# tum-pbs/DMCF

Hardware: AMD Instinct MI355X
Metric: rollout_particle_steps_per_sec (higher is better)
Workload: dtype f32

## Files before the change

dmcf_amd/_lib.py:

```python
import ctypes
import os
import subprocess

_PKG = os.path.dirname(os.path.abspath(__file__))
LIB_PATH = os.path.join(_PKG, "libdmcf_hip.so")
_lib = None


class DmcfError(RuntimeError):
    pass


class CconvArgs(ctypes.Structure):
    _fields_ = [
        ("filters", ctypes.c_void_p),
        ("filter_dims", ctypes.c_int32 * 5),
        ("sym_axis", ctypes.c_int32),
        ("out_positions", ctypes.c_void_p),
        ("n_out", ctypes.c_int64),
        ("inp_positions", ctypes.c_void_p),
        ("n_inp", ctypes.c_int64),
        ("inp_features", ctypes.c_void_p),
        ("inp_importance", ctypes.c_void_p),
        ("neighbors_index", ctypes.c_void_p),
        ("neighbors_row_splits", ctypes.c_void_p),
        ("neighbors_value", ctypes.c_void_p),
        ("extent", ctypes.c_float),
        ("window_fac", ctypes.c_float),
        ("window", ctypes.c_int32),
        ("coordinate_mapping", ctypes.c_int32),
        ("interpolation", ctypes.c_int32),
        ("flags", ctypes.c_int32),
        ("bias", ctypes.c_void_p),
        ("out", ctypes.c_void_p),
        ("n_pairs", ctypes.c_int64),
        ("neighbors_row_count", ctypes.c_void_p),
        ("filter_tile_mask", ctypes.c_uint32),
        ("row_length_hint", ctypes.c_int32),
    ]


class CconvBackwardArgs(ctypes.Structure):
    _fields_ = [
        ("struct_size", ctypes.c_uint32),
        ("flags", ctypes.c_int32),
        ("grad_out", ctypes.c_void_p),
        ("inv_index", ctypes.c_void_p),
        ("inv_pair", ctypes.c_void_p),
        ("inv_row_splits", ctypes.c_void_p),
        ("inv_n_rows", ctypes.c_int64),
        ("inv_n_pairs", ctypes.c_int64),
        ("grad_filters", ctypes.c_void_p),
        ("grad_inp_features", ctypes.c_void_p),
    ]


class NeighborDenseArgs(ctypes.Structure):
    _fields_ = [
        ("struct_size", ctypes.c_uint32),
        ("flags", ctypes.c_int32),
        ("x", ctypes.c_void_p),
        ("n_in", ctypes.c_int64),
        ("cin", ctypes.c_int32),
        ("cout", ctypes.c_int32),
        ("kernel", ctypes.c_void_p),
        ("bias", ctypes.c_void_p),
        ("residual", ctypes.c_void_p),
        ("mask", ctypes.c_void_p),
        ("neighbors_index", ctypes.c_void_p),
        ("neighbors_row_splits", ctypes.c_void_p),
        ("neighbors_row_count", ctypes.c_void_p),
        ("n_out", ctypes.c_int64),
        ("n_pairs", ctypes.c_int64),
        ("host_row_splits", ctypes.c_void_p),
        ("out", ctypes.c_void_p),
        ("record_s", ctypes.c_void_p),
        ("record_count", ctypes.c_void_p),
    ]


class NeighborDenseBackwardArgs(ctypes.Structure):
    _fields_ = [
        ("struct_size", ctypes.c_uint32),
        ("flags", ctypes.c_int32),
        ("x", ctypes.c_void_p),
        ("n_in", ctypes.c_int64),
        ("cin", ctypes.c_int32),
        ("cout", ctypes.c_int32),
        ("kernel", ctypes.c_void_p),
        ("grad_out", ctypes.c_void_p),
        ("n_out", ctypes.c_int64),
        ("s", ctypes.c_void_p),
        ("count", ctypes.c_void_p),
        ("inv_index", ctypes.c_void_p),
        ("inv_row_splits", ctypes.c_void_p),
        ("inv_n_pairs", ctypes.c_int64),
        ("grad_x", ctypes.c_void_p),
        ("grad_kernel", ctypes.c_void_p),
        ("grad_bias", ctypes.c_void_p),
    ]


class LatticeConvArgs(ctypes.Structure):
    _fields_ = [
        ("filters", ctypes.c_void_p),
        ("filter_dims", ctypes.c_int32 * 5),
        ("inp_volume", ctypes.c_void_p),
        ("inp_min", ctypes.c_int32 * 3),
        ("inp_dims", ctypes.c_int32 * 3),
        ("out_table", ctypes.c_void_p),
        ("out_min", ctypes.c_int32 * 3),
        ("out_dims", ctypes.c_int32 * 3),
        ("n_out", ctypes.c_int64),
        ("inp_step", ctypes.c_int32),
        ("out_stride", ctypes.c_int32),
        ("out_phase", ctypes.c_int32 * 3),
        ("base_min", ctypes.c_int32 * 3),
        ("base_dims", ctypes.c_int32 * 3),
        ("rel_shift", ctypes.c_float * 3),
        ("voxel", ctypes.c_float * 3),
        ("offsets", ctypes.c_void_p),
        ("n_offsets", ctypes.c_int64),
        ("reach", ctypes.c_int32 * 3),
        ("extent", ctypes.c_float),
        ("window_fac", ctypes.c_float),
        ("window", ctypes.c_int32),
        ("coordinate_mapping", ctypes.c_int32),
        ("interpolation", ctypes.c_int32),
        ("flags", ctypes.c_int32),
        ("bias", ctypes.c_void_p),
        ("out", ctypes.c_void_p),
    ]


class CconvScatterArgs(ctypes.Structure):
    _fields_ = [
        ("filters", ctypes.c_void_p),
        ("filter_dims", ctypes.c_int32 * 5),
        ("out_positions", ctypes.c_void_p),
        ("n_out", ctypes.c_int64),
        ("inp_positions", ctypes.c_void_p),
        ("n_inp", ctypes.c_int64),
        ("inp_features", ctypes.c_void_p),
        ("t_index", ctypes.c_void_p),
        ("t_row_begin", ctypes.c_void_p),
        ("t_row_count", ctypes.c_void_p),
        ("t_capacity", ctypes.c_int64),
        ("plan", ctypes.c_void_p),
        ("block_cells", ctypes.c_int32),
        ("reach", ctypes.c_int32),
        ("extent", ctypes.c_float),
        ("window_fac", ctypes.c_float),
        ("window", ctypes.c_int32),
        ("flags", ctypes.c_int32),
        ("bias", ctypes.c_void_p),
        ("out", ctypes.c_void_p),
        ("error_flag", ctypes.c_void_p),
    ]


class AdamTensor(ctypes.Structure):
    _fields_ = [
        ("param", ctypes.c_void_p),
        ("grad", ctypes.c_void_p),
        ("m", ctypes.c_void_p),
        ("v", ctypes.c_void_p),
        ("n", ctypes.c_int64),
    ]


class AdamArgs(ctypes.Structure):
    _fields_ = [
        ("struct_size", ctypes.c_uint32),
        ("n_tensors", ctypes.c_int32),
        ("tensors", ctypes.c_void_p),
        ("device_tensors", ctypes.c_void_p),
        ("lr", ctypes.c_float),
        ("beta_1", ctypes.c_float),
        ("beta_2", ctypes.c_float),
        ("epsilon", ctypes.c_float),
        ("beta_1_power", ctypes.c_float),
        ("beta_2_power", ctypes.c_float),
        ("clip_norm", ctypes.c_float),
        ("reserved", ctypes.c_int32),
    ]


class Sph1dParams(ctypes.Structure):
    _fields_ = [
        ("struct_size", ctypes.c_uint32),
        ("bcnt", ctypes.c_int32),
        ("max_iter", ctypes.c_int32),
        ("reserved", ctypes.c_int32),
        ("h", ctypes.c_double),
        ("rest_dens", ctypes.c_double),
        ("stiffness", ctypes.c_double),
        ("visc", ctypes.c_double),
        ("gravity", ctypes.c_double),
        ("dt", ctypes.c_double),
        ("eps", ctypes.c_double),
    ]


SYMBOLS = [
    "dmcf_version", "dmcf_error_string", "dmcf_last_hip_error",
    "dmcf_frs_workspace_bytes", "dmcf_frs_build", "dmcf_frs_count", "dmcf_frs_write", "dmcf_frs_search_padded", "dmcf_frs_window_sum",
    "dmcf_radius_search_count", "dmcf_radius_search_write",
    "dmcf_cconv_workspace_bytes", "dmcf_cconv_forward", "dmcf_cconv_kernel_name",
    "dmcf_cconv_forward_extents", "dmcf_cconv_extents_kernel_name",
    "dmcf_invert_neighbors_list_workspace_bytes", "dmcf_invert_neighbors_list",
    "dmcf_cconv_backward_workspace_bytes", "dmcf_cconv_backward", "dmcf_cconv_backward_kernel_names",
    "dmcf_cconv_backward_extents", "dmcf_cconv_backward_extents_kernel_names",
    "dmcf_cconv_scatter_plan_bytes", "dmcf_cconv_scatter_plan", "dmcf_cconv_scatter_workspace_bytes", "dmcf_cconv_scatter_forward",
    "dmcf_lattice_conv_workspace_bytes", "dmcf_lattice_conv_forward",
    "dmcf_lattice_conv_batch_workspace_bytes", "dmcf_lattice_conv_forward_batch",
    "dmcf_lattice_conv_backward_workspace_bytes", "dmcf_lattice_conv_backward",
    "dmcf_reduce_subarrays_sum", "dmcf_points_aabb_workspace_bytes", "dmcf_points_aabb", "dmcf_dense_forward",
    "dmcf_fps_workspace_bytes", "dmcf_farthest_point_sample", "dmcf_gather_point",
    "dmcf_grid_pos_workspace_bytes", "dmcf_grid_pos_bounds", "dmcf_grid_pos_count", "dmcf_grid_pos_write",
    "dmcf_ghost_workspace_bytes", "dmcf_ghost_count", "dmcf_ghost_write",
    "dmcf_nn_distance_workspace_bytes", "dmcf_nn_distance", "dmcf_approx_match_workspace_bytes", "dmcf_approx_match",
    "dmcf_match_cost_workspace_bytes", "dmcf_match_cost", "dmcf_emd_workspace_bytes", "dmcf_emd",
    "dmcf_neighbor_dense_forward", "dmcf_neighbor_dense_backward_workspace_bytes", "dmcf_neighbor_dense_backward",
    "dmcf_neighbor_dense_kernel_names", "dmcf_adam_step_workspace_bytes", "dmcf_adam_step", "dmcf_adam_step_kernel_names",
    "dmcf_raster_workspace_bytes", "dmcf_raster_count", "dmcf_raster_discs",
    "dmcf_nn_distance_backward_workspace_bytes", "dmcf_nn_distance_backward", "dmcf_match_cost_backward_workspace_bytes",
    "dmcf_match_cost_backward", "dmcf_emd_with_levels", "dmcf_emd_backward_workspace_bytes", "dmcf_emd_backward",
    "dmcf_gather_point_backward_workspace_bytes", "dmcf_gather_point_backward",
    "dmcf_frs_window_sum_backward",
    "dmcf_sph1d_rollout",
]


def build(force=False):
    csrc = os.path.join(_PKG, "csrc")
    args = ["make", "-C", csrc, "-j4"]
    if force:
        args.append("-B")
    subprocess.check_call(args, stdout=subprocess.DEVNULL)
    return LIB_PATH


def lib():
    global _lib
    if _lib is not None:
        return _lib
    if not os.path.exists(LIB_PATH):
        raise DmcfError(
            f"{LIB_PATH} is missing: the HIP extension has not been built "
            "(run `python -c 'import __graft_entry__ as g; g.build()'`). There is no CPU fallback.")
    L = ctypes.CDLL(LIB_PATH)
    c = ctypes
    L.dmcf_version.restype = c.c_int
    L.dmcf_error_string.restype = c.c_char_p
    L.dmcf_error_string.argtypes = [c.c_int]
    L.dmcf_last_hip_error.restype = c.c_int
    L.dmcf_frs_workspace_bytes.restype = c.c_size_t
    L.dmcf_frs_workspace_bytes.argtypes = [c.c_int64, c.c_int64]
    L.dmcf_frs_build.restype = c.c_int
    L.dmcf_frs_build.argtypes = [c.c_void_p, c.c_int64, c.c_float, c.c_void_p, c.c_size_t, c.c_void_p]
    L.dmcf_frs_count.restype = c.c_int
    L.dmcf_frs_count.argtypes = [c.c_void_p, c.c_int64, c.c_int64, c.c_float, c.c_int, c.c_void_p, c.c_size_t,
                                 c.c_void_p, c.c_void_p]
    L.dmcf_frs_write.restype = c.c_int
    L.dmcf_frs_write.argtypes = [c.c_void_p, c.c_int64, c.c_int64, c.c_float, c.c_int, c.c_void_p, c.c_size_t,
                                 c.c_void_p, c.c_void_p, c.c_void_p, c.c_int64, c.c_void_p]
    L.dmcf_frs_search_padded.restype = c.c_int
    L.dmcf_frs_search_padded.argtypes = [c.c_void_p, c.c_int64, c.c_int64, c.c_float, c.c_int, c.c_void_p, c.c_size_t, c.c_int64,
                                         c.c_void_p, c.c_void_p, c.c_void_p, c.c_void_p, c.c_void_p, c.c_void_p]
    L.dmcf_frs_window_sum.restype = c.c_int
    L.dmcf_frs_window_sum.argtypes = [c.c_void_p, c.c_int64, c.c_int64, c.c_float, c.c_int, c.c_int, c.c_void_p, c.c_size_t,
                                      c.c_void_p, c.c_void_p]
    L.dmcf_radius_search_count.restype = c.c_int
    L.dmcf_radius_search_count.argtypes = [c.c_void_p, c.c_int64, c.c_int64, c.c_void_p, c.c_float, c.c_int, c.c_void_p, c.c_size_t,
                                           c.c_void_p, c.c_void_p]
    L.dmcf_radius_search_write.restype = c.c_int
    L.dmcf_radius_search_write.argtypes = [c.c_void_p, c.c_int64, c.c_int64, c.c_void_p, c.c_float, c.c_int, c.c_void_p, c.c_size_t,
                                           c.c_void_p, c.c_void_p, c.c_void_p, c.c_int64, c.c_void_p]
    L.dmcf_cconv_workspace_bytes.restype = c.c_size_t
    L.dmcf_cconv_workspace_bytes.argtypes = [c.POINTER(CconvArgs)]
    L.dmcf_cconv_forward.restype = c.c_int
    L.dmcf_cconv_forward.argtypes = [c.POINTER(CconvArgs), c.c_void_p, c.c_size_t, c.c_void_p]
    L.dmcf_cconv_kernel_name.restype = c.c_int
    L.dmcf_cconv_kernel_name.argtypes = [c.POINTER(CconvArgs), c.c_char_p, c.c_size_t]
    L.dmcf_cconv_forward_extents.restype = c.c_int
    L.dmcf_cconv_forward_extents.argtypes = [c.POINTER(CconvArgs), c.c_void_p, c.c_void_p, c.c_size_t, c.c_void_p]
    L.dmcf_cconv_extents_kernel_name.restype = c.c_int
    L.dmcf_cconv_extents_kernel_name.argtypes = [c.POINTER(CconvArgs), c.c_char_p, c.c_size_t]
    L.dmcf_invert_neighbors_list_workspace_bytes.restype = c.c_size_t
    L.dmcf_invert_neighbors_list_workspace_bytes.argtypes = [c.c_int64]
    L.dmcf_invert_neighbors_list.restype = c.c_int
    L.dmcf_invert_neighbors_list.argtypes = [c.c_int64, c.c_void_p, c.c_void_p, c.c_void_p, c.c_int64, c.c_int64, c.c_void_p,
                                             c.c_void_p, c.c_void_p, c.c_void_p, c.c_void_p, c.c_void_p, c.c_size_t, c.c_void_p]
    L.dmcf_cconv_backward_workspace_bytes.restype = c.c_size_t
    L.dmcf_cconv_backward_workspace_bytes.argtypes = [c.POINTER(CconvArgs), c.POINTER(CconvBackwardArgs)]
    L.dmcf_cconv_backward.restype = c.c_int
    L.dmcf_cconv_backward.argtypes = [c.POINTER(CconvArgs), c.POINTER(CconvBackwardArgs), c.c_void_p, c.c_size_t, c.c_void_p]
    L.dmcf_cconv_backward_kernel_names.restype = c.c_int
    L.dmcf_cconv_backward_kernel_names.argtypes = [c.POINTER(CconvArgs), c.POINTER(CconvBackwardArgs), c.c_char_p, c.c_size_t]
    L.dmcf_cconv_backward_extents.restype = c.c_int
    L.dmcf_cconv_backward_extents.argtypes = [c.POINTER(CconvArgs), c.POINTER(CconvBackwardArgs), c.c_void_p, c.c_void_p, c.c_size_t,
                                              c.c_void_p]
    L.dmcf_cconv_backward_extents_kernel_names.restype = c.c_int
    L.dmcf_cconv_backward_extents_kernel_names.argtypes = [c.POINTER(CconvArgs), c.POINTER(CconvBackwardArgs), c.c_char_p, c.c_size_t]
    L.dmcf_cconv_scatter_plan_bytes.restype = c.c_size_t
    L.dmcf_cconv_scatter_plan_bytes.argtypes = [c.c_int64]
    L.dmcf_cconv_scatter_plan.restype = c.c_int
    L.dmcf_cconv_scatter_plan.argtypes = [c.c_void_p, c.c_int64, c.c_void_p, c.c_int64, c.c_float, c.c_float, c.c_int32, c.c_void_p,
                                          c.c_size_t, c.c_void_p]
    L.dmcf_cconv_scatter_workspace_bytes.restype = c.c_size_t
    L.dmcf_cconv_scatter_workspace_bytes.argtypes = [c.POINTER(CconvScatterArgs)]
    L.dmcf_cconv_scatter_forward.restype = c.c_int
    L.dmcf_cconv_scatter_forward.argtypes = [c.POINTER(CconvScatterArgs), c.c_void_p, c.c_size_t, c.c_void_p]
    L.dmcf_lattice_conv_workspace_bytes.restype = c.c_size_t
    L.dmcf_lattice_conv_workspace_bytes.argtypes = [c.POINTER(LatticeConvArgs)]
    L.dmcf_lattice_conv_forward.restype = c.c_int
    L.dmcf_lattice_conv_forward.argtypes = [c.POINTER(LatticeConvArgs), c.c_void_p, c.c_size_t, c.c_void_p]
    L.dmcf_lattice_conv_batch_workspace_bytes.restype = c.c_size_t
    L.dmcf_lattice_conv_batch_workspace_bytes.argtypes = [c.POINTER(LatticeConvArgs), c.c_int32]
    L.dmcf_lattice_conv_forward_batch.restype = c.c_int
    L.dmcf_lattice_conv_forward_batch.argtypes = [c.POINTER(LatticeConvArgs), c.c_int32, c.c_void_p, c.c_size_t, c.c_void_p]
    L.dmcf_lattice_conv_backward_workspace_bytes.restype = c.c_size_t
    L.dmcf_lattice_conv_backward_workspace_bytes.argtypes = [c.POINTER(LatticeConvArgs), c.c_int32]
    L.dmcf_lattice_conv_backward.restype = c.c_int
    L.dmcf_lattice_conv_backward.argtypes = [c.POINTER(LatticeConvArgs), c.c_int32, c.c_void_p, c.c_void_p, c.c_void_p, c.c_void_p,
                                             c.c_size_t, c.c_void_p]
    L.dmcf_dense_forward.restype = c.c_int
    L.dmcf_dense_forward.argtypes = [c.c_void_p, c.c_int64, c.c_int32, c.c_void_p, c.c_int32, c.c_void_p, c.c_void_p, c.c_void_p,
                                     c.c_void_p]
    L.dmcf_ghost_workspace_bytes.restype = c.c_size_t
    L.dmcf_ghost_workspace_bytes.argtypes = [c.c_int64, c.c_int32, c.c_int32]
    L.dmcf_ghost_count.restype = c.c_int
    L.dmcf_ghost_count.argtypes = [c.c_void_p, c.c_int64, c.c_void_p, c.c_int32, c.c_void_p, c.c_int32, c.c_void_p, c.c_void_p,
                                   c.c_size_t, c.c_void_p]
    L.dmcf_ghost_write.restype = c.c_int
    L.dmcf_ghost_write.argtypes = [c.c_void_p, c.c_int64, c.c_void_p, c.c_int32, c.c_void_p, c.c_int32, c.c_void_p, c.c_void_p,
                                   c.c_void_p, c.c_void_p, c.c_size_t, c.c_void_p]
    L.dmcf_points_aabb_workspace_bytes.restype = c.c_size_t
    L.dmcf_points_aabb_workspace_bytes.argtypes = []
    L.dmcf_points_aabb.restype = c.c_int
    L.dmcf_points_aabb.argtypes = [c.c_void_p, c.c_int64, c.c_void_p, c.c_void_p, c.c_size_t, c.c_void_p]
    L.dmcf_reduce_subarrays_sum.restype = c.c_int
    L.dmcf_reduce_subarrays_sum.argtypes = [c.c_void_p, c.c_void_p, c.c_int64, c.c_void_p, c.c_void_p]
    L.dmcf_fps_workspace_bytes.restype = c.c_size_t
    L.dmcf_fps_workspace_bytes.argtypes = [c.c_int64]
    L.dmcf_farthest_point_sample.restype = c.c_int
    L.dmcf_farthest_point_sample.argtypes = [c.c_void_p, c.c_int64, c.c_int64, c.c_void_p, c.c_size_t, c.c_void_p, c.c_void_p]
    L.dmcf_gather_point.restype = c.c_int
    L.dmcf_gather_point.argtypes = [c.c_void_p, c.c_void_p, c.c_int64, c.c_int, c.c_void_p, c.c_void_p]
    L.dmcf_grid_pos_workspace_bytes.restype = c.c_size_t
    L.dmcf_grid_pos_workspace_bytes.argtypes = [c.c_int64]
    f3 = c.POINTER(c.c_float)
    L.dmcf_grid_pos_bounds.restype = c.c_int
    L.dmcf_grid_pos_bounds.argtypes = [c.c_void_p, c.c_int64, f3, c.c_int, c.c_void_p, c.c_int, c.c_float, c.c_void_p,
                                       c.c_size_t, c.c_void_p]
    L.dmcf_grid_pos_count.restype = c.c_int
    L.dmcf_grid_pos_count.argtypes = [c.c_void_p, c.c_int64, f3, c.c_int, c.c_int, c.c_float, c.c_void_p, c.c_size_t,
                                      c.c_void_p, c.c_int64, c.c_void_p]
    L.dmcf_grid_pos_write.restype = c.c_int
    L.dmcf_grid_pos_write.argtypes = [c.c_void_p, c.c_int64, f3, c.c_int, c.c_int, c.c_float, c.c_void_p, c.c_size_t,
                                      c.c_void_p, c.c_int64, c.c_void_p, c.c_int64, c.c_void_p]
    for q in ("dmcf_nn_distance_workspace_bytes", "dmcf_approx_match_workspace_bytes", "dmcf_match_cost_workspace_bytes",
              "dmcf_emd_workspace_bytes"):
        getattr(L, q).restype = c.c_size_t
        getattr(L, q).argtypes = [c.c_int64, c.c_int64, c.c_int64]
    L.dmcf_nn_distance.restype = c.c_int
    L.dmcf_nn_distance.argtypes = [c.c_void_p, c.c_void_p, c.c_int64, c.c_int64, c.c_int64, c.c_void_p, c.c_void_p, c.c_void_p,
                                   c.c_void_p, c.c_void_p, c.c_size_t, c.c_void_p]
    i32p = c.POINTER(c.c_int32)
    for f in ("dmcf_approx_match", "dmcf_emd"):
        getattr(L, f).restype = c.c_int
        getattr(L, f).argtypes = [c.c_void_p, c.c_void_p, c.c_int64, c.c_int64, c.c_int64, i32p, i32p, c.c_void_p, c.c_void_p,
                                  c.c_size_t, c.c_void_p]
    L.dmcf_match_cost.restype = c.c_int
    L.dmcf_match_cost.argtypes = [c.c_void_p, c.c_void_p, c.c_int64, c.c_int64, c.c_int64, c.c_void_p, c.c_void_p, c.c_void_p,
                                  c.c_size_t, c.c_void_p]
    L.dmcf_neighbor_dense_forward.restype = c.c_int
    L.dmcf_neighbor_dense_forward.argtypes = [c.POINTER(NeighborDenseArgs), c.c_void_p]
    L.dmcf_neighbor_dense_backward_workspace_bytes.restype = c.c_size_t
    L.dmcf_neighbor_dense_backward_workspace_bytes.argtypes = [c.POINTER(NeighborDenseBackwardArgs)]
    L.dmcf_neighbor_dense_backward.restype = c.c_int
    L.dmcf_neighbor_dense_backward.argtypes = [c.POINTER(NeighborDenseBackwardArgs), c.c_void_p, c.c_size_t, c.c_void_p]
    L.dmcf_neighbor_dense_kernel_names.restype = c.c_int
    L.dmcf_neighbor_dense_kernel_names.argtypes = [c.POINTER(NeighborDenseArgs), c.POINTER(NeighborDenseBackwardArgs), c.c_char_p,
                                                   c.c_size_t]
    L.dmcf_adam_step_workspace_bytes.restype = c.c_size_t
    L.dmcf_adam_step_workspace_bytes.argtypes = [c.POINTER(AdamArgs)]
    L.dmcf_adam_step.restype = c.c_int
    L.dmcf_adam_step.argtypes = [c.POINTER(AdamArgs), c.c_void_p, c.c_size_t, c.c_void_p]
    L.dmcf_adam_step_kernel_names.restype = c.c_int
    L.dmcf_adam_step_kernel_names.argtypes = [c.POINTER(AdamArgs), c.c_char_p, c.c_size_t]
    L.dmcf_raster_workspace_bytes.restype = c.c_size_t
    L.dmcf_raster_workspace_bytes.argtypes = [c.c_int64, c.c_int64, c.c_int64, c.c_int32, c.c_int32]
    L.dmcf_raster_count.restype = c.c_int
    L.dmcf_raster_count.argtypes = [c.c_void_p, c.c_int64, c.c_int64, c.c_int64, c.c_float, c.c_int32, c.c_int32, c.c_void_p, c.c_size_t,
                                    c.c_void_p, c.c_void_p]
    L.dmcf_raster_discs.restype = c.c_int
    L.dmcf_raster_discs.argtypes = [c.c_void_p, c.c_int64, c.c_int64, c.c_int64, c.c_float, c.c_uint32, c.c_int32, c.c_int32, c.c_void_p,
                                    c.c_void_p, c.c_size_t, c.c_void_p, c.c_int64, c.c_void_p]
    for q in ("dmcf_nn_distance_backward_workspace_bytes", "dmcf_match_cost_backward_workspace_bytes",
              "dmcf_emd_backward_workspace_bytes"):
        getattr(L, q).restype = c.c_size_t
        getattr(L, q).argtypes = [c.c_int64, c.c_int64, c.c_int64]
    L.dmcf_nn_distance_backward.restype = c.c_int
    L.dmcf_nn_distance_backward.argtypes = [c.c_void_p, c.c_void_p, c.c_int64, c.c_int64, c.c_int64, c.c_void_p, c.c_void_p,
                                            c.c_void_p, c.c_void_p, c.c_void_p, c.c_void_p, c.c_void_p, c.c_size_t, c.c_void_p]
    L.dmcf_match_cost_backward.restype = c.c_int
    L.dmcf_match_cost_backward.argtypes = [c.c_void_p, c.c_void_p, c.c_int64, c.c_int64, c.c_int64, c.c_void_p, c.c_void_p,
                                           c.c_void_p, c.c_void_p, c.c_void_p, c.c_size_t, c.c_void_p]
    L.dmcf_emd_with_levels.restype = c.c_int
    L.dmcf_emd_with_levels.argtypes = [c.c_void_p, c.c_void_p, c.c_int64, c.c_int64, c.c_int64, i32p, i32p, c.c_void_p, c.c_void_p,
                                       c.c_void_p, c.c_size_t, c.c_void_p]
    L.dmcf_emd_backward.restype = c.c_int
    L.dmcf_emd_backward.argtypes = [c.c_void_p, c.c_void_p, c.c_int64, c.c_int64, c.c_int64, i32p, i32p, c.c_void_p, c.c_void_p,
                                    c.c_void_p, c.c_void_p, c.c_void_p, c.c_size_t, c.c_void_p]
    L.dmcf_gather_point_backward_workspace_bytes.restype = c.c_size_t
    L.dmcf_gather_point_backward_workspace_bytes.argtypes = [c.c_int64, c.c_int64]
    L.dmcf_gather_point_backward.restype = c.c_int
    L.dmcf_gather_point_backward.argtypes = [c.c_void_p, c.c_void_p, c.c_int64, c.c_int, c.c_int64, c.c_void_p, c.c_void_p,
                                             c.c_size_t, c.c_void_p]
    L.dmcf_frs_window_sum_backward.restype = c.c_int
    L.dmcf_frs_window_sum_backward.argtypes = [c.c_void_p, c.c_int64, c.c_int64, c.c_float, c.c_int, c.c_int, c.c_void_p, c.c_void_p,
                                               c.c_void_p, c.c_size_t, c.c_void_p, c.c_void_p]
    L.dmcf_sph1d_rollout.restype = c.c_int
    L.dmcf_sph1d_rollout.argtypes = [c.c_void_p, c.c_void_p, c.c_int64, c.c_int32, c.POINTER(Sph1dParams), c.c_int32, c.c_void_p,
                                     c.c_void_p, c.c_void_p, c.c_void_p]
    _lib = L
    return L


def check(rc, what):
    if rc != 0:
        L = lib()
        raise DmcfError(f"{what}: {L.dmcf_error_string(rc).decode()} (code {rc}, hip error {L.dmcf_last_hip_error()})")
```

dmcf_amd/csrc/cconv_lat.hip:

```cpp
#include "cconv_common.h"

namespace dmcf {

struct LatParams {
    const float* Wp;
    const int32_t* stencil;
    int S, KS, NT, cin, cout;
    const float* vol;
    int imin[3], idim[3];
    const int32_t* otab;
    int omin[3], odim[3];
    int inp_step, out_stride, phase[3];
    int amin[3], adim[3];
    int tiles_x;
    int64_t ntiles;
    const float* bias;
    float* out;
    int flags;
};

typedef int lat_i32x2 __attribute__((ext_vector_type(2)));
constexpr int kLatMaxParts = 8;
constexpr int kLatRowsPerGroup = 128;
constexpr int kLatCellsPerBlock = 1024;
struct LatBatch {
    LatParams part[kLatMaxParts];
    int64_t cfirst[kLatMaxParts + 1];
    int n;
    uint32_t* blk;
    int64_t* start;
    int64_t* count;
    lat_i32x2* rows;
    int64_t rows_capacity;
};

__device__ __forceinline__ int lat_cell(const LatParams& p, int64_t c, int& rowb) {
    const int64_t tile = c >> 4;
    const int m = (int)(c & 15);
    rowb = 0;
    if (tile >= p.ntiles) return -1;
    const int xb = (int)(tile % p.tiles_x);
    const int ax = p.amin[0] + xb * 16 + m, ay = p.amin[1] + (int)(tile / p.tiles_x % p.adim[1]),
              az = p.amin[2] + (int)(tile / ((int64_t)p.tiles_x * p.adim[1]));
    const int ox = ax * p.out_stride + p.phase[0] - p.omin[0], oy = ay * p.out_stride + p.phase[1] - p.omin[1],
              oz = az * p.out_stride + p.phase[2] - p.omin[2];
    if (!(xb * 16 + m < p.adim[0] && (unsigned)ox < (unsigned)p.odim[0] && (unsigned)oy < (unsigned)p.odim[1] &&
          (unsigned)oz < (unsigned)p.odim[2]))
        return -1;
    const int ix = ax * p.inp_step - p.imin[0], iy = ay * p.inp_step - p.imin[1], iz = az * p.inp_step - p.imin[2];
    rowb = ((iz * p.idim[1] + iy) * p.idim[0] + ix) * p.cin * 4;
    return p.otab[((int64_t)oz * p.odim[1] + oy) * p.odim[0] + ox];
}

__device__ __forceinline__ int lat_part_of_block(const LatBatch& b, int64_t block) {
    int i = 0;
    while (i + 1 < b.n && block >= b.cfirst[i + 1]) ++i;
    return i;
}

__global__ __launch_bounds__(256) void lat_rows_count(const LatBatch b) {
    __shared__ uint32_t wsum[4];
    const int i = lat_part_of_block(b, blockIdx.x);
    const int64_t c0 = ((int64_t)blockIdx.x - b.cfirst[i]) * kLatCellsPerBlock;
    uint32_t mine = 0;
    for (int r = 0; r < kLatCellsPerBlock / 256; ++r) {
        int rowb;
        mine += (uint32_t)__popcll(__ballot(lat_cell(b.part[i], c0 + r * 256 + threadIdx.x, rowb) >= 0));
    }
    if ((threadIdx.x & 63) == 0) wsum[threadIdx.x >> 6] = mine;
    __syncthreads();
    if (threadIdx.x == 0) {
        b.blk[blockIdx.x] = wsum[0] + wsum[1] + wsum[2] + wsum[3];
        if (blockIdx.x == 0) b.blk[b.cfirst[b.n]] = 0;
    }
}

__global__ void lat_rows_starts(const LatBatch b) {
    if (threadIdx.x != 0) return;
    int64_t s = 0;
    for (int i = 0; i < b.n; ++i) {
        const int64_t n = (int64_t)b.blk[b.cfirst[i + 1]] - (int64_t)b.blk[b.cfirst[i]];
        b.start[i] = s;
        b.count[i] = n;
        s += (n + kLatRowsPerGroup - 1) / kLatRowsPerGroup * kLatRowsPerGroup;
    }
    b.start[b.n] = s;
}

__global__ __launch_bounds__(256) void lat_rows_write(const LatBatch b) {
    __shared__ uint32_t wsum[4];
    const int i = lat_part_of_block(b, blockIdx.x);
    const int64_t c0 = ((int64_t)blockIdx.x - b.cfirst[i]) * kLatCellsPerBlock;
    const int lane = threadIdx.x & 63, wave = threadIdx.x >> 6;
    int64_t at = b.start[i] + ((int64_t)b.blk[blockIdx.x] - (int64_t)b.blk[b.cfirst[i]]);
    for (int r = 0; r < kLatCellsPerBlock / 256; ++r) {
        int rowb;
        const int oi = lat_cell(b.part[i], c0 + r * 256 + threadIdx.x, rowb);
        const uint64_t mk = __ballot(oi >= 0);
        if (lane == 0) wsum[wave] = (uint32_t)__popcll(mk);
        __syncthreads();
        if (oi >= 0) {
            int64_t pos = at + __popcll(mk & ((1ull << lane) - 1ull));
            for (int v = 0; v < wave; ++v) pos += wsum[v];
            if (pos < b.rows_capacity) b.rows[pos] = (lat_i32x2){rowb, oi};
        }
        at += wsum[0] + wsum[1] + wsum[2] + wsum[3];
        __syncthreads();
    }
}

struct LatTaps {
    float a;
    int bx, by, bz;
    float wx[2], wy[2], wz[2];
};
__device__ __forceinline__ LatTaps lat_offset_taps(const int32_t* __restrict__ stencil, int s, const CconvParams& p, float vx, float vy,
                                                   float vz, float sx, float sy, float sz) {
    LatTaps g;
    float x = (float)stencil[4 * s] * vx - sx, y = (float)stencil[4 * s + 1] * vy - sy, z = (float)stencil[4 * s + 2] * vz - sz;
    const float d2 = (x * x + y * y) + z * z;
    g.a = window_value(p.window, d2, p.inv_r2, p.window_fac);
    filter_coords<true>(x, y, z, p);
    axis_weights(x, p.sx, p.interp, g.bx, g.wx[0], g.wx[1]);
    axis_weights(y, p.sy, p.interp, g.by, g.wy[0], g.wy[1]);
    axis_weights(z, p.sz, p.interp, g.bz, g.wz[0], g.wz[1]);
    return g;
}

__global__ __launch_bounds__(256) void lat_build_filters(const float* __restrict__ W, float* __restrict__ Wp,
                                                         const int32_t* __restrict__ stencil, int S, int KS, int NT, CconvParams p,
                                                         float vx, float vy, float vz, float sx, float sy, float sz) {
    const int64_t total = (int64_t)((S + 3) / 4) * 4 * KS * NT * 64;
    for (int64_t e = (int64_t)blockIdx.x * blockDim.x + threadIdx.x; e < total; e += (int64_t)gridDim.x * blockDim.x) {
        int64_t t = e;
        const int n = (int)(t & 15); t >>= 4;
        const int q = (int)(t & 3); t >>= 2;
        const int nt = (int)(t % NT); t /= NT;
        const int c = (int)(t % (4 * KS)); t /= 4 * KS;
        const int s = (int)t * 4 + q, o = nt * 16 + n;
        float v = 0.0f;
        if (s < S && c < p.cin && o < p.cout) {
            const LatTaps g = lat_offset_taps(stencil, s, p, vx, vy, vz, sx, sy, sz);
            for (int iz = 0; iz < 2; ++iz)
                for (int iy = 0; iy < 2; ++iy)
                    for (int ix = 0; ix < 2; ++ix) {
                        const float w = g.wz[iz] * g.wy[iy] * g.wx[ix];
                        if (w == 0.0f) continue;
                        const int cz = min(g.bz + iz, p.sz - 1), cy = min(g.by + iy, p.sy - 1), cx = min(g.bx + ix, p.sx - 1);
                        v += w * W[((((int64_t)cz * p.sy + cy) * p.sx + cx) * p.cin + c) * p.cout + o];
                    }
            v *= g.a;
        }
        Wp[e] = v;
    }
}

constexpr int kLatTW = 2;
constexpr int kLatCH = 32;
constexpr int kLatG = kLatCH / 4;
static_assert(kLatRowsPerGroup == 4 * kLatTW * 16, "rows of a workgroup");

template <int NTT, int KST>
__device__ __forceinline__ void lat_conv_body(const LatParams& p, const lat_i32x2* __restrict__ rows, const int64_t first, const int64_t end) {
    __shared__ __attribute__((aligned(16))) float Ws[2][kLatCH * KST * NTT * 64];
    const int lane = threadIdx.x & 63, wave = threadIdx.x >> 6;
    const int m = lane & 15, q = lane >> 4;
    constexpr int C = 4 * KST;
    int oidx[kLatTW];
    int rowb[kLatTW];
    f32x4 acc[kLatTW][NTT];
    bool any = false;
#pragma unroll
    for (int t = 0; t < kLatTW; ++t) {
        const int64_t e = first + ((wave * kLatTW + t) << 4) + m;
        oidx[t] = -1;
        rowb[t] = (((p.amin[2] * p.inp_step - p.imin[2]) * p.idim[1] + (p.amin[1] * p.inp_step - p.imin[1])) * p.idim[0] +
                   (p.amin[0] * p.inp_step - p.imin[0])) * p.cin * 4;
        if (e < end) {
            const lat_i32x2 rw = rows[e];
            rowb[t] = rw.x;
            oidx[t] = rw.y;
        }
        if (__ballot(oidx[t] >= 0) == 0) oidx[t] = -2;
        any |= oidx[t] != -2;
#pragma unroll
        for (int n = 0; n < NTT; ++n) acc[t][n] = (f32x4){0.0f, 0.0f, 0.0f, 0.0f};
    }
    if (!__syncthreads_or(any ? 1 : 0)) return;
    typedef int i32x4 __attribute__((ext_vector_type(4)));
    const int NG = (p.S + 3) / 4;
    constexpr int kQuads = kLatCH * KST * NTT * 64 / 4 / 256;
    f32x4 wr[kQuads];
    i32x4 dv;
    auto fetch = [&](int s0) {
        const int g0 = s0 / 4, ng = min(kLatG, NG - g0);
#pragma unroll
        for (int i = 0; i < kQuads; ++i) {
            const int e = (threadIdx.x + 256 * i) * 4;
            const int l = e & 63, n = (e >> 6) % NTT, gc = (e >> 6) / NTT;
            wr[i] = (gc < ng * C && n < p.NT) ? *(const f32x4*)(p.Wp + (((int64_t)g0 * C + gc) * p.NT + n) * 64 + l)
                                              : (f32x4){0.0f, 0.0f, 0.0f, 0.0f};
        }
        dv = *(const i32x4*)(p.stencil + 4 * min(s0 + (lane & (kLatCH - 1)), p.S - 1));
    };
    auto stash = [&](int buf) {
#pragma unroll
        for (int i = 0; i < kQuads; ++i) *(f32x4*)(Ws[buf] + (threadIdx.x + 256 * i) * 4) = wr[i];
    };
    fetch(0);
    stash(0);
    __syncthreads();
    for (int s0 = 0, k = 0; s0 < p.S; s0 += kLatCH, ++k) {
        const int ng = min(kLatG, NG - s0 / 4);
        const float* Wc = Ws[k & 1];
        const int dof = ((dv.z * p.idim[1] + dv.y) * p.idim[0] + dv.x) * p.cin * 4;
        int dofg[kLatG];
#pragma unroll
        for (int g = 0; g < kLatG; ++g) dofg[g] = __shfl(dof, 4 * g + q, 64);
        const bool more = s0 + kLatCH < p.S;
        if (more) fetch(s0 + kLatCH);
        if (any) {
            f32x4 f[3][kLatTW][KST];
            auto gather = [&](int g, f32x4 (&fv)[kLatTW][KST]) {
#pragma unroll
                for (int t = 0; t < kLatTW; ++t) {
                    const f32x4* src = (const f32x4*)((const char*)p.vol + (size_t)(uint32_t)(rowb[t] + dofg[g]));
#pragma unroll
                    for (int ks = 0; ks < KST; ++ks) fv[t][ks] = src[ks];
                }
            };
            auto products = [&](int g, const f32x4 (&fv)[kLatTW][KST]) {
#pragma unroll
                for (int c = 0; c < C; ++c)
#pragma unroll
                    for (int n = 0; n < NTT; ++n) {
                        const float w = Wc[((g * C + c) * NTT + n) * 64 + lane];
#pragma unroll
                        for (int t = 0; t < kLatTW; ++t)
                            acc[t][n] = __builtin_amdgcn_mfma_f32_16x16x4f32(fv[t][c >> 2][c & 3], w, acc[t][n], 0, 0, 0);
                    }
            };
            gather(0, f[0]);
            gather(1, f[1]);
#pragma unroll
            for (int g = 0; g < kLatG; ++g) {
                if (g >= ng) break;
                if (g + 2 < kLatG) gather(g + 2, f[(g + 2) % 3]);
                products(g, f[g % 3]);
            }
        }
        if (more) stash((k + 1) & 1);
        __syncthreads();
    }
#pragma unroll
    for (int t = 0; t < kLatTW; ++t) {
        if (oidx[t] == -2) continue;
#pragma unroll
        for (int r = 0; r < 4; ++r) {
            const int oi = __shfl(oidx[t], 4 * q + r, 64);
            if (oi < 0) continue;
#pragma unroll
            for (int n = 0; n < NTT; ++n) {
                const int o = 16 * n + m;
                if (o >= p.cout) continue;
                float v = acc[t][n][r];
                if (p.bias) v += p.bias[o];
                float* dst = p.out + (int64_t)oi * p.cout + o;
                if (p.flags & DMCF_FLAG_ACCUMULATE) v += *dst;
                *dst = v;
            }
        }
    }
}

template <int NTT, int KST>
__global__ __launch_bounds__(256) void lat_conv_kernel(const LatBatch b) {
    const int64_t first = (int64_t)blockIdx.x * kLatRowsPerGroup;
    if (first >= b.start[b.n]) return;
    int i = 0;
    while (i + 1 < b.n && first >= b.start[i + 1]) ++i;
    lat_conv_body<NTT, KST>(b.part[i], b.rows, first, b.start[i] + b.count[i]);
}

static size_t lat_packed_floats(const dmcf_lattice_conv_args* a) {
    const int KS = (a->filter_dims[3] + 3) / 4, NT = (a->filter_dims[4] + 15) / 16;
    return (size_t)((a->n_offsets + 3) / 4) * 4 * KS * NT * 64;
}

static int lat_validate(const dmcf_lattice_conv_args* a) {
    if (!a) return DMCF_EINVAL;
    for (int k = 0; k < 5; ++k)
        if (a->filter_dims[k] <= 0) return DMCF_EINVAL;
    if (a->n_out < 0 || a->n_offsets < 0 || a->inp_step <= 0 || a->out_stride <= 0 || !(a->extent > 0.0f)) return DMCF_EINVAL;
    if (a->n_out > 0 && (!a->filters || !a->out_table || !a->out || !a->inp_volume || (a->n_offsets > 0 && !a->offsets)))
        return DMCF_EINVAL;
    for (int k = 0; k < 3; ++k)
        if (a->inp_dims[k] <= 0 || a->out_dims[k] <= 0 || a->base_dims[k] <= 0 || !(a->voxel[k] >= 0.0f)) return DMCF_EINVAL;
    if (a->flags & (DMCF_FLAG_SYMMETRIC | DMCF_FLAG_NORMALIZE)) return DMCF_EUNSUPPORTED;
    if (a->window == DMCF_WINDOW_EXPLICIT) return DMCF_EUNSUPPORTED;
    const int cin = a->filter_dims[3], cout = a->filter_dims[4];
    if ((cin != 4 && cin != 8) || cout > 32) return DMCF_EUNSUPPORTED;
    return DMCF_OK;
}

}

namespace dmcf {

static CconvParams lat_cconv_params(const dmcf_lattice_conv_args* a) {
    CconvParams cp = {};
    cp.sz = a->filter_dims[0]; cp.sy = a->filter_dims[1]; cp.sx = a->filter_dims[2];
    cp.K = cp.sx * cp.sy * cp.sz;
    cp.cin = a->filter_dims[3]; cp.cout = a->filter_dims[4];
    cp.inv_extent = 1.0f / a->extent;
    const float radius = 0.5f * a->extent;
    cp.inv_r2 = 1.0f / (radius * radius);
    cp.window_fac = a->window_fac;
    cp.window = a->window;
    cp.mapping = a->coordinate_mapping;
    cp.interp = a->interpolation;
    cp.flags = a->flags;
    return cp;
}

static int lat_prepare(const dmcf_lattice_conv_args* a, float* packed, hipStream_t stream, LatParams& p, int64_t& groups) {
    const int cin = a->filter_dims[3], cout = a->filter_dims[4];
    const int KS = (cin + 3) / 4, NT = (cout + 15) / 16;
    for (int k = 0; k < 3; ++k) {
        const int64_t ext = k == 0 ? (int64_t)((a->base_dims[0] + 15) / 16) * 16 : a->base_dims[k];
        const int64_t lo = (int64_t)a->base_min[k] * a->inp_step - a->reach[k];
        const int64_t hi = ((int64_t)a->base_min[k] + ext - 1) * a->inp_step + a->reach[k];
        if (a->reach[k] < 0 || lo < a->inp_min[k] || hi > (int64_t)a->inp_min[k] + a->inp_dims[k] - 1) return DMCF_EINVAL;
    }
    if ((int64_t)a->inp_dims[0] * a->inp_dims[1] * a->inp_dims[2] * cin > 0x1fffffff) return DMCF_EUNSUPPORTED;
    const CconvParams cp = lat_cconv_params(a);
    if (a->n_offsets > 0) {
        const int64_t total = (int64_t)lat_packed_floats(a);
        const unsigned g = (unsigned)((total + 255) / 256);
        hipLaunchKernelGGL(lat_build_filters, dim3(g < 4096u ? g : 4096u), dim3(256), 0, stream, a->filters, packed, a->offsets,
                           (int)a->n_offsets, KS, NT, cp, a->voxel[0], a->voxel[1], a->voxel[2], a->rel_shift[0], a->rel_shift[1],
                           a->rel_shift[2]);
    }
    p.Wp = packed;
    p.stencil = a->offsets;
    p.S = (int)a->n_offsets; p.KS = KS; p.NT = NT; p.cin = cin; p.cout = cout;
    p.vol = a->inp_volume;
    p.otab = a->out_table;
    for (int k = 0; k < 3; ++k) {
        p.imin[k] = a->inp_min[k]; p.idim[k] = a->inp_dims[k];
        p.omin[k] = a->out_min[k]; p.odim[k] = a->out_dims[k];
        p.phase[k] = a->out_phase[k];
        p.amin[k] = a->base_min[k];
        p.adim[k] = a->base_dims[k];
    }
    p.inp_step = a->inp_step;
    p.out_stride = a->out_stride;
    p.tiles_x = (a->base_dims[0] + 15) / 16;
    p.ntiles = (int64_t)p.tiles_x * a->base_dims[1] * a->base_dims[2];
    p.bias = a->bias; p.out = a->out; p.flags = a->flags;
    groups = (p.ntiles * 16 + kLatCellsPerBlock - 1) / kLatCellsPerBlock;
    return DMCF_OK;
}

struct LatLayout {
    size_t off_blk, off_scan, off_tmp, tmp_bytes, off_start, off_rows, total;
    int64_t nblk, rows_capacity;
};

static LatLayout lat_layout(const dmcf_lattice_conv_args* parts, int n_parts) {
    LatLayout L;
    size_t off = 256;
    L.nblk = 0;
    for (int i = 0; i < n_parts; ++i) {
        off += align_up(lat_packed_floats(parts + i) * sizeof(float), 256);
        const int64_t cells = (int64_t)((parts[i].base_dims[0] + 15) / 16) * 16 * parts[i].base_dims[1] * parts[i].base_dims[2];
        L.nblk += (cells + kLatCellsPerBlock - 1) / kLatCellsPerBlock;
    }
    L.off_blk = off;    off += align_up((size_t)(L.nblk + 1) * 4, 256);
    L.off_scan = off;   off += align_up((size_t)(L.nblk + 1) * 4, 256);
    L.tmp_bytes = scan_tmp_bytes(L.nblk + 1);
    L.off_tmp = off;    off += align_up(L.tmp_bytes, 256);
    L.off_start = off;  off += 256;
    L.rows_capacity = (parts[0].n_out + kLatRowsPerGroup - 1) / kLatRowsPerGroup * kLatRowsPerGroup + (int64_t)kLatRowsPerGroup * n_parts;
    L.off_rows = off;   off += align_up((size_t)L.rows_capacity * sizeof(lat_i32x2), 256);
    L.total = off;
    return L;
}

static int lat_check(const dmcf_lattice_conv_args* parts, int n_parts) {
    for (int i = 0; i < n_parts; ++i) {
        const int rc = lat_validate(parts + i);
        if (rc != DMCF_OK) return rc;
        if (parts[i].filter_dims[3] != parts[0].filter_dims[3] || parts[i].filter_dims[4] != parts[0].filter_dims[4] ||
            parts[i].n_out != parts[0].n_out || parts[i].out != parts[0].out)
            return DMCF_EINVAL;
    }
    return DMCF_OK;
}

static int lat_rows(const dmcf_lattice_conv_args* parts, int n_parts, void* workspace, size_t workspace_bytes, size_t need,
                    hipStream_t stream, LatBatch& b, const LatLayout& L) {
    if (!workspace || ((uintptr_t)workspace & 255)) return DMCF_EINVAL;
    if (workspace_bytes < need) return DMCF_EWORKSPACE;
    if (L.nblk > 0x7ffffffe) return DMCF_EUNSUPPORTED;
    b.n = n_parts;
    char* ws = (char*)workspace;
    char* wp = ws;
    int64_t first = 0;
    for (int i = 0; i < n_parts; ++i) {
        int64_t blocks;
        const int rc = lat_prepare(parts + i, (float*)wp, stream, b.part[i], blocks);
        if (rc != DMCF_OK) return rc;
        wp += align_up(lat_packed_floats(parts + i) * sizeof(float), 256);
        b.cfirst[i] = first;
        first += blocks;
    }
    for (int i = n_parts; i <= kLatMaxParts; ++i) b.cfirst[i] = first;
    if (first != L.nblk) return DMCF_EINVAL;
    uint32_t* blk_in = (uint32_t*)(ws + L.off_blk);
    b.blk = blk_in;
    b.start = (int64_t*)(ws + L.off_start);
    b.count = b.start + kLatMaxParts + 1;
    b.rows = (lat_i32x2*)(ws + L.off_rows);
    b.rows_capacity = L.rows_capacity;
    hipLaunchKernelGGL(lat_rows_count, dim3((unsigned)L.nblk), dim3(256), 0, stream, b);
    const int rc = scan_exclusive_u32(blk_in, (uint32_t*)(ws + L.off_scan), L.nblk + 1, ws + L.off_tmp, L.tmp_bytes, stream);
    if (rc != DMCF_OK) return rc;
    b.blk = (uint32_t*)(ws + L.off_scan);
    hipLaunchKernelGGL(lat_rows_starts, dim3(1), dim3(64), 0, stream, b);
    hipLaunchKernelGGL(lat_rows_write, dim3((unsigned)L.nblk), dim3(256), 0, stream, b);
    return DMCF_OK;
}

static int lat_launch(const dmcf_lattice_conv_args* parts, int n_parts, void* workspace, size_t workspace_bytes, hipStream_t stream) {
    int rc = lat_check(parts, n_parts);
    if (rc != DMCF_OK) return rc;
    if (parts[0].n_out == 0) return DMCF_OK;
    const LatLayout L = lat_layout(parts, n_parts);
    LatBatch b;
    rc = lat_rows(parts, n_parts, workspace, workspace_bytes, L.total, stream, b, L);
    if (rc != DMCF_OK) return rc;
    const dim3 grid((unsigned)(L.rows_capacity / kLatRowsPerGroup)), block(256);
    const int KS = b.part[0].KS, NT = b.part[0].NT;
    if (KS == 1 && NT == 1) hipLaunchKernelGGL((lat_conv_kernel<1, 1>), grid, block, 0, stream, b);
    else if (KS == 1) hipLaunchKernelGGL((lat_conv_kernel<2, 1>), grid, block, 0, stream, b);
    else if (NT == 1) hipLaunchKernelGGL((lat_conv_kernel<1, 2>), grid, block, 0, stream, b);
    else hipLaunchKernelGGL((lat_conv_kernel<2, 2>), grid, block, 0, stream, b);
    return check_launch();
}

#include "cconv_lat_bwd.inc"

}

using namespace dmcf;

extern "C" {

size_t dmcf_lattice_conv_workspace_bytes(const dmcf_lattice_conv_args* a) {
    if (lat_validate(a) != DMCF_OK) return 256;
    return lat_layout(a, 1).total;
}

size_t dmcf_lattice_conv_batch_workspace_bytes(const dmcf_lattice_conv_args* parts, int32_t n_parts) {
    if (!parts || n_parts < 1 || n_parts > kLatMaxParts) return 256;
    for (int i = 0; i < n_parts; ++i)
        if (lat_validate(parts + i) != DMCF_OK) return 256;
    return lat_layout(parts, n_parts).total;
}

int dmcf_lattice_conv_forward(const dmcf_lattice_conv_args* a, void* workspace, size_t workspace_bytes, dmcf_stream_t stream_) {
    if (!a) return DMCF_EINVAL;
    return lat_launch(a, 1, workspace, workspace_bytes, (hipStream_t)stream_);
}

int dmcf_lattice_conv_forward_batch(const dmcf_lattice_conv_args* parts, int32_t n_parts, void* workspace, size_t workspace_bytes,
                                    dmcf_stream_t stream_) {
    if (!parts || n_parts < 1 || n_parts > kLatMaxParts) return DMCF_EINVAL;
    return lat_launch(parts, n_parts, workspace, workspace_bytes, (hipStream_t)stream_);
}

size_t dmcf_lattice_conv_backward_workspace_bytes(const dmcf_lattice_conv_args* parts, int32_t n_parts) {
    dmcf_lattice_conv_args own[kLatMaxParts];
    if (lat_bwd_parts(parts, n_parts, own) != DMCF_OK) return 256;
    return lat_bwd_layout(own, n_parts).total;
}

int dmcf_lattice_conv_backward(const dmcf_lattice_conv_args* parts, int32_t n_parts, const float* grad_out, float* grad_volume,
                               float* grad_filters, void* workspace, size_t workspace_bytes, dmcf_stream_t stream_) {
    return lat_backward(parts, n_parts, grad_out, grad_volume, grad_filters, workspace, workspace_bytes, (hipStream_t)stream_);
}

}
```

dmcf_amd/csrc/misc.hip:

```cpp
#include "common.h"

namespace dmcf {

thread_local int g_last_hip_error = 0;

constexpr int kScanThreads = 256;
constexpr int kScanItems = 8;
constexpr int kScanTile = kScanThreads * kScanItems;

template <typename T>
__device__ __forceinline__ T wave_inclusive_scan(T v) {
#pragma unroll
    for (int d = 1; d < kWave; d <<= 1) {
        T o = __shfl_up(v, d, kWave);
        if (lane_id() >= d) v += o;
    }
    return v;
}

template <typename T>
__device__ __forceinline__ T block_exclusive_scan(T v, T* total, T* smem ) {
    const int wave = threadIdx.x >> 6;
    const T inc = wave_inclusive_scan(v);
    if (lane_id() == kWave - 1) smem[wave] = inc;
// ... 88 lines not shown
int scan_exclusive_u32(const uint32_t* in, uint32_t* out, int64_t n, void* tmp, size_t tmp_bytes,
                       hipStream_t stream) {
    return scan_impl<uint32_t, uint32_t, false>(in, out, n, tmp, tmp_bytes, stream);
}

int scan_counts_to_row_splits(const int32_t* counts, int64_t* row_splits, int64_t n, void* tmp,
                              size_t tmp_bytes, hipStream_t stream) {
    return scan_impl<int32_t, int64_t, true>(counts, row_splits, n, tmp, tmp_bytes, stream);
}

typedef float dense_f32x4 __attribute__((ext_vector_type(4)));
template <int NT>
__global__ __launch_bounds__(256) void dense_rows(const float* __restrict__ x, int64_t n, int k, const float* __restrict__ W, int m,
                                                  const float* __restrict__ bias, const float* __restrict__ residual,
                                                  float* __restrict__ out, int64_t ntiles) {
    const int lane = lane_id(), r = lane & 15, q = lane >> 4;
    const int kj = (k + 15) >> 4;
    float wf[4][4][NT];
#pragma unroll
    for (int j = 0; j < 4; ++j)
#pragma unroll
        for (int i = 0; i < 4; ++i)
#pragma unroll
            for (int t = 0; t < NT; ++t) {
                const int kk = 16 * j + 4 * q + i, col = 16 * t + r;
                wf[j][i][t] = (kk < k && col < m) ? W[(size_t)kk * m + col] : 0.0f;
            }
    float bs[NT];
#pragma unroll
    for (int t = 0; t < NT; ++t) bs[t] = (bias && 16 * t + r < m) ? bias[16 * t + r] : 0.0f;
    const int64_t wave = (int64_t)blockIdx.x * 4 + (threadIdx.x >> 6), nwaves = (int64_t)gridDim.x * 4;
    for (int64_t tile = wave; tile < ntiles; tile += nwaves) {
        const int64_t row = tile * 16 + r;
        dense_f32x4 a[4];
#pragma unroll
        for (int j = 0; j < 4; ++j) {
            a[j] = (dense_f32x4){0.0f, 0.0f, 0.0f, 0.0f};
            if (j < kj && row < n && 16 * j + 4 * q < k) a[j] = *(const dense_f32x4*)(x + row * k + 16 * j + 4 * q);
        }
        dense_f32x4 acc[NT];
#pragma unroll
        for (int t = 0; t < NT; ++t) acc[t] = (dense_f32x4){0.0f, 0.0f, 0.0f, 0.0f};
#pragma unroll
        for (int j = 0; j < 4; ++j) {
            if (j < kj) {
#pragma unroll
                for (int i = 0; i < 4; ++i)
#pragma unroll
                    for (int t = 0; t < NT; ++t) acc[t] = __builtin_amdgcn_mfma_f32_16x16x4f32(a[j][i], wf[j][i][t], acc[t], 0, 0, 0);
            }
        }
#pragma unroll
        for (int rr = 0; rr < 4; ++rr) {
            const int64_t orow = tile * 16 + 4 * q + rr;
            if (orow >= n) continue;
#pragma unroll
            for (int t = 0; t < NT; ++t) {
                const int col = 16 * t + r;
                if (col >= m) continue;
                float v = acc[t][rr] + bs[t];
                if (residual) v += residual[orow * m + col];
                out[orow * m + col] = v;
            }
        }
    }
}

constexpr int kAabbBlocks = 1024;

__global__ __launch_bounds__(256) void aabb_partial(const float* __restrict__ pts, int64_t n, float* __restrict__ part) {
    float mn[3] = {INFINITY, INFINITY, INFINITY}, mx[3] = {-INFINITY, -INFINITY, -INFINITY};
    bool bad[3] = {false, false, false};
    for (int64_t i = (int64_t)blockIdx.x * 256 + threadIdx.x; i < n; i += (int64_t)gridDim.x * 256) {
#pragma unroll
        for (int a = 0; a < 3; ++a) {
            const float v = pts[3 * i + a];
            mn[a] = fminf(mn[a], v);
            mx[a] = fmaxf(mx[a], v);
            bad[a] |= v != v;
        }
    }
    __shared__ float red[3][3][4];
#pragma unroll
    for (int a = 0; a < 3; ++a) {
        float b = bad[a] ? 1.0f : 0.0f;
#pragma unroll
        for (int d = 32; d >= 1; d >>= 1) {
            mn[a] = fminf(mn[a], __shfl_xor(mn[a], d, kWave));
            mx[a] = fmaxf(mx[a], __shfl_xor(mx[a], d, kWave));
            b = fmaxf(b, __shfl_xor(b, d, kWave));
        }
        if (lane_id() == 0) {
            red[0][a][threadIdx.x >> 6] = mn[a];
            red[1][a][threadIdx.x >> 6] = mx[a];
            red[2][a][threadIdx.x >> 6] = b;
        }
    }
    __syncthreads();
    if (threadIdx.x < 3) {
        const int a = threadIdx.x;
        float* o = part + (size_t)blockIdx.x * 8;
        const bool b = fmaxf(fmaxf(red[2][a][0], red[2][a][1]), fmaxf(red[2][a][2], red[2][a][3])) > 0.0f;
        o[a] = b ? NAN : fminf(fminf(red[0][a][0], red[0][a][1]), fminf(red[0][a][2], red[0][a][3]));
        o[3 + a] = b ? NAN : fmaxf(fmaxf(red[1][a][0], red[1][a][1]), fmaxf(red[1][a][2], red[1][a][3]));
    }
}

__global__ void aabb_finish(const float* __restrict__ part, int nblocks, float* __restrict__ out) {
    const int lane = lane_id();
#pragma unroll
    for (int a = 0; a < 3; ++a) {
        float mn = INFINITY, mx = -INFINITY, b = 0.0f;
        for (int k = lane; k < nblocks; k += kWave) {
            const float lo = part[(size_t)k * 8 + a], hi = part[(size_t)k * 8 + 3 + a];
            b = fmaxf(b, lo != lo ? 1.0f : 0.0f);
            mn = fminf(mn, lo);
            mx = fmaxf(mx, hi);
        }
#pragma unroll
        for (int d = 32; d >= 1; d >>= 1) {
            mn = fminf(mn, __shfl_xor(mn, d, kWave));
            mx = fmaxf(mx, __shfl_xor(mx, d, kWave));
            b = fmaxf(b, __shfl_xor(b, d, kWave));
        }
        if (lane == 0) {
            out[a] = b > 0.0f ? NAN : mn;
            out[3 + a] = b > 0.0f ? NAN : mx;
        }
    }
}

__global__ __launch_bounds__(256) void reduce_subarrays_sum_kernel(const float* __restrict__ values,
                                                                   const int64_t* __restrict__ row_splits,
                                                                   int64_t n_rows, float* __restrict__ out) {
    const int64_t row = ((int64_t)blockIdx.x * blockDim.x + threadIdx.x) >> 4;
    const int sub = threadIdx.x & 15;
    if (row >= n_rows) return;
    const int64_t b = row_splits[row], e = row_splits[row + 1];
    float s = 0.0f;
    if (values) {
        for (int64_t k = b + sub; k < e; k += 16) s += values[k];
    } else {
        for (int64_t k = b + sub; k < e; k += 16) s += 1.0f;
    }
#pragma unroll
    for (int d = 8; d >= 1; d >>= 1) s += __shfl_xor(s, d, 16);
    if (sub == 0) out[row] = s;
}

}

extern "C" {

int dmcf_version(void) { return 21700; }

const char* dmcf_error_string(int code) {
    switch (code) {
        case DMCF_OK: return "ok";
        case DMCF_EINVAL: return "invalid argument";
        case DMCF_EWORKSPACE: return "workspace too small";
        case DMCF_ELAUNCH: return "HIP error while enqueuing (see dmcf_last_hip_error)";
        case DMCF_EUNSUPPORTED: return "option not implemented on the HIP path";
        default: return "unknown error code";
    }
}

int dmcf_last_hip_error(void) { return dmcf::g_last_hip_error; }

int dmcf_dense_forward(const float* x, int64_t n, int32_t k, const float* W, int32_t m, const float* bias,
                       const float* residual, float* out, dmcf_stream_t stream) {
    if (n < 0 || k <= 0 || m <= 0 || (n > 0 && (!x || !W || !out))) return DMCF_EINVAL;
    if ((k & 3) || k > 64 || m > 64) return DMCF_EUNSUPPORTED;
    if ((uintptr_t)x & 15) return DMCF_EUNSUPPORTED;
    if (n == 0) return DMCF_OK;
    const int64_t ntiles = (n + 15) / 16;
    const int64_t want = (ntiles + 3) / 4;
    const unsigned grid = (unsigned)(want < 2048 ? want : 2048);
    const int nt = (m + 15) / 16;
#define DMCF_DENSE(NTT)                                                                                                   \
    hipLaunchKernelGGL(dmcf::dense_rows<NTT>, dim3(grid), dim3(256), 0, (hipStream_t)stream, x, n, (int)k, W, (int)m, bias,  \
                       residual, out, ntiles)
    if (nt <= 1) DMCF_DENSE(1);
    else if (nt == 2) DMCF_DENSE(2);
    else DMCF_DENSE(4);
#undef DMCF_DENSE
    return dmcf::check_launch();
}

size_t dmcf_points_aabb_workspace_bytes(void) { return (size_t)dmcf::kAabbBlocks * 8 * sizeof(float); }

int dmcf_points_aabb(const float* points, int64_t n, float* out, void* workspace, size_t workspace_bytes,
                     dmcf_stream_t stream) {
    if (n < 0 || !out || (n > 0 && !points)) return DMCF_EINVAL;
    if (!workspace || workspace_bytes < dmcf_points_aabb_workspace_bytes()) return DMCF_EWORKSPACE;
    const int64_t want = (n + 1023) / 1024;
    const int nb = (int)(want < 1 ? 1 : (want > dmcf::kAabbBlocks ? dmcf::kAabbBlocks : want));
    hipLaunchKernelGGL(dmcf::aabb_partial, dim3(nb), dim3(256), 0, (hipStream_t)stream, points, n, (float*)workspace);
    hipLaunchKernelGGL(dmcf::aabb_finish, dim3(1), dim3(64), 0, (hipStream_t)stream, (const float*)workspace, nb, out);
    return dmcf::check_launch();
}

int dmcf_reduce_subarrays_sum(const float* values, const int64_t* row_splits, int64_t n_rows, float* out,
                              dmcf_stream_t stream) {
    if (n_rows < 0 || (n_rows > 0 && (!row_splits || !out))) return DMCF_EINVAL;
    if (n_rows == 0) return DMCF_OK;
    const int64_t threads = n_rows * 16;
    const unsigned grid = (unsigned)((threads + 255) / 256);
    hipLaunchKernelGGL(dmcf::reduce_subarrays_sum_kernel, dim3(grid), dim3(256), 0, (hipStream_t)stream, values,
                       row_splits, n_rows, out);
    return dmcf::check_launch();
}

}
```

dmcf_amd/lattice.py:

```python
import collections
import os
import threading

import numpy as np
import torch

_TLS = threading.local()
_KEEP = 16

MAX_X_OVER_EXTENT = float(os.environ.get("DMCF_LATTICE_MAX_RATIO", "32"))
MAX_VOLUME_FLOATS = 1 << 28
MAX_CELLS_PER_POINT = 32
CORE_MIN_FILL = float(os.environ.get("DMCF_LATTICE_CORE_FILL", str(1.0 / 32)))
CORE_SLAB_FRACTION = 0.125
_FAR = 3.0e4


def _registry():
    r = getattr(_TLS, "registry", None)
    if r is None:
        r = _TLS.registry = collections.OrderedDict()
    return r


def clear():
    _registry().clear()


def _cores():
    r = getattr(_TLS, "cores", None)
    if r is None:
        r = _TLS.cores = {}
    return r


def _pick_core(minp, dims, hists):
    lo, hi = [], []
    for k in range(3):
        h = hists[k]
        m = max(h) if h else 0
        if m <= 0:
            lo.append(minp[k]); hi.append(minp[k] + dims[k])
            continue
        thr = CORE_SLAB_FRACTION * m
        peak = h.index(m)
        a = b = peak
        gap = 0
        i = peak - 1
        while i >= 0 and gap <= 2:
            if h[i] >= thr:
                a, gap = i, 0
            else:
                gap += 1
            i -= 1
        gap = 0
        i = peak + 1
        while i < len(h) and gap <= 2:
            if h[i] >= thr:
                b, gap = i, 0
            else:
                gap += 1
            i += 1
        lo.append(minp[k] + a); hi.append(minp[k] + b + 1)
    return lo, hi


class LatticeInfo:
    def __init__(self, gpos, center, voxel, family, minp, dims, keep=None, center_host=None):
        self.gpos = gpos
        self.max_abs = None
        if center_host is not None:
            self.max_abs = max(abs(float(center_host[k])) + max(abs(int(minp[k])), abs(int(minp[k]) + int(dims[k]))) * float(voxel[k])
                               for k in range(3))
        self.keep = keep
        self.version = gpos._version
        self.center = center
        self.voxel = tuple(float(np.float32(v)) for v in voxel)
        self.family = family
        self.minp = [int(v) for v in minp]
        self.dims = [int(v) for v in dims]
        self._cells = None
        self._lin = None
        self._vlin = {}
        self._table = None
        self._core = None
        self._tables = {}

    def cells(self):
        if self._cells is None:
            v = torch.tensor(self.voxel, dtype=torch.float32, device=self.gpos.device)
            self._cells = torch.round((self.gpos - self.center) / v).to(torch.int32).contiguous()
        return self._cells

    def lin(self, minp=None, dims=None):
        own = minp is None
        if own and self._lin is not None:
            return self._lin
        minp, dims = (self.minp, self.dims) if own else (minp, dims)
        dx, dy, dz = dims
        c = self.cells().long()
        lin = ((c[:, 2] - minp[2]) * dy + (c[:, 1] - minp[1])) * dx + (c[:, 0] - minp[0])
        if os.environ.get("DMCF_LATTICE_CHECK") == "1":
            lo = torch.tensor(list(minp), device=c.device)
            hi = lo + torch.tensor(list(dims), device=c.device)
            if not bool(((c >= lo) & (c < hi)).all()):
                raise RuntimeError("lattice points outside the registered box of cells")
        if own:
            self._lin = lin
        return lin

    def core(self):
        if self._core is not None:
            return self._core
        n = self.gpos.shape[0]
        dx, dy, dz = self.dims
        whole = (list(self.minp), list(self.dims), None, None, None)
        if n / float(dx * dy * dz) >= CORE_MIN_FILL or os.environ.get("DMCF_LATTICE_CORE", "1") == "0":
            self._core = whole
            return whole
        from .utils.convolutions import _CACHE
        dev = self.gpos.device
        c = self.cells()
        minp, dims = list(self.minp), list(self.dims)
        lo_box = torch.tensor(minp, dtype=torch.int32, device=dev)
        rel = torch.minimum((c - lo_box).long().clamp_(min=0), torch.tensor(dims, device=dev) - 1)
        hist = torch.cat([torch.bincount(rel[:, k], minlength=dims[k])[: dims[k]] for k in range(3)])
        key = (_CACHE.key, self.voxel)

        def split(h):
            return [h[: dx], h[dx: dx + dy], h[dx + dy:]]

        def next_entry(h):
            hs = split(h)
            lo, hi = _pick_core(minp, dims, hs)
            bound = sum(n - sum(hs[k][lo[k] - minp[k]: hi[k] - minp[k]]) for k in range(3))
            return dict(box=(lo, hi), cap=int(2 * bound + 65536))

        est = _cores().get(key) if (_CACHE.depth > 0 and _CACHE.use_hints) else None
        if est is None:
            est = next_entry(hist.tolist())
            exact = True
        else:
            exact = False
        lo = [max(est["box"][0][k], minp[k]) for k in range(3)]
        hi = [min(est["box"][1][k], minp[k] + dims[k]) for k in range(3)]
        if any(hi[k] <= lo[k] for k in range(3)):
            lo, hi = minp, [minp[k] + dims[k] for k in range(3)]
        lo_t = torch.tensor(lo, dtype=torch.int32, device=dev)
        hi_t = torch.tensor(hi, dtype=torch.int32, device=dev)
        outside = ~((c >= lo_t) & (c < hi_t)).all(dim=1)
        count = outside.sum().reshape(1)
        if exact:
            m = int(count.item())
            _cores()[key] = est
            valid = None
        else:
            m = min(est["cap"], n)
            cap = m

            def report(vals):
                _cores()[key] = next_entry(vals[1:])
                return vals[0] > cap
            _CACHE.report(torch.cat([count, hist]), report)
        if m == 0:
            idx = pos = valid = None
        else:
            idx = torch.nonzero_static(outside, size=m, fill_value=-1).flatten()
            if not exact:
                valid = (idx >= 0).to(torch.float32).unsqueeze(1)
                idx = idx.clamp(min=0)
            pos = self.gpos.index_select(0, idx).contiguous()
            if valid is not None:
                far = max(_FAR, 4.0 * (self.max_abs or 0.0) + 1.0e3)
                pos = torch.where(valid > 0, pos, torch.full_like(pos, far))
        self._core = (lo, [hi[k] - lo[k] for k in range(3)], idx, pos, valid)
        return self._core

    def table_in(self, minp, dims):
        key = (tuple(minp), tuple(dims))
        t = self._tables.get(key)
        if t is None:
            dx, dy, dz = dims
            c = self.cells().long()
            lo = torch.tensor(list(minp), device=c.device)
            hi = lo + torch.tensor(list(dims), device=c.device)
            ok = ((c >= lo) & (c < hi)).all(dim=1)
            lin = ((c[:, 2] - minp[2]) * dy + (c[:, 1] - minp[1])) * dx + (c[:, 0] - minp[0])
            lin = torch.where(ok, lin, torch.full_like(lin, dz * dy * dx))
            t = torch.full((dz * dy * dx + 1,), -1, dtype=torch.int32, device=c.device)
            t[lin] = torch.where(ok, torch.arange(c.shape[0], dtype=torch.int32, device=c.device), torch.full((1,), -1, dtype=torch.int32, device=c.device))
            t = self._tables[key] = t[:-1].view(dz, dy, dx)
        return t

    def volume_in(self, features, minp, dims):
        key = ("in", tuple(minp), tuple(dims))
        lin = self._vlin.get(key)
        dx, dy, dz = dims
        if lin is None:
            c = self.cells().long()
            lo = torch.tensor(list(minp), device=c.device)
            hi = lo + torch.tensor(list(dims), device=c.device)
            ok = ((c >= lo) & (c < hi)).all(dim=1)
            lin = ((c[:, 2] - minp[2]) * dy + (c[:, 1] - minp[1])) * dx + (c[:, 0] - minp[0])
            lin = self._vlin[key] = torch.where(ok, lin, torch.full_like(lin, dz * dy * dx))
        v = features.new_zeros((dz * dy * dx + 1, features.shape[1]))
        v[lin] = features
        return v[:-1].view(dz, dy, dx, features.shape[1])

    def table(self):
        if self._table is None:
            dx, dy, dz = self.dims
            t = torch.full((dz * dy * dx,), -1, dtype=torch.int32, device=self.gpos.device)
            t[self.lin()] = torch.arange(self.gpos.shape[0], dtype=torch.int32, device=self.gpos.device)
            self._table = t.view(dz, dy, dx)
        return self._table

    def volume(self, features, minp=None, dims=None):
        key = None if minp is None else (tuple(minp), tuple(dims))
        lin = self._vlin.get(key)
        if lin is None:
            lin = self._vlin[key] = self.lin(minp, dims)
        dx, dy, dz = self.dims if minp is None else dims
        v = features.new_zeros((dz * dy * dx, features.shape[1]))
        v[lin] = features
        return v.view(dz, dy, dx, features.shape[1])


def register(gpos, center, voxel, family, minp, dims, keep=None, center_host=None):
    if gpos.shape[0] == 0 or any(not (float(v) > 1e-5) for v in voxel):
        return
    reg = _registry()
    reg[(gpos.data_ptr(), gpos.shape[0])] = LatticeInfo(gpos, center, voxel, family, minp, dims, keep, center_host)
    while len(reg) > _KEEP:
        reg.popitem(last=False)


def register_points(pos, center, voxel, family, box=None, keep=None, center_host=None):
    if pos.shape[0] == 0 or any(not (float(v) > 1e-5) for v in voxel) or not pos.is_cuda:
        return
    if box is None:
        v = torch.tensor([float(np.float32(x)) for x in voxel], dtype=torch.float32, device=pos.device)
        cells = torch.round((pos - center) / v).to(torch.int32)
        lo, hi = cells.amin(dim=0), cells.amax(dim=0)
        b = torch.cat([lo, hi - lo + 1]).tolist()
        box = (b[0:3], b[3:6])
    info = LatticeInfo(pos, center, voxel, family, box[0], box[1], keep if keep is not None else center, center_host)
    reg = _registry()
    reg[(pos.data_ptr(), pos.shape[0])] = info
    while len(reg) > _KEEP:
        reg.popitem(last=False)


def lookup(t):
    info = _registry().get((t.data_ptr(), t.shape[0]))
    if info is None or info.gpos._version != info.version or t.dim() != 2 or t.dtype != torch.float32 or not t.is_contiguous():
        return None
    return info


def enabled():
    from . import ops
    return os.environ.get("DMCF_LATTICE_CONV", "1") != "0" and ops.search_set() == "distance"


class LatticePair:

    def __init__(self, inp, out, ratio):
        self.inp, self.out, self.ratio = inp, out, ratio

    def plan(self, ops, extent, dev):
        key = (float(extent), str(dev))
        hit = getattr(self, "_plan", None)
        if hit is not None and hit[0] == key:
            return hit[1]
        a, b = self.inp, self.out
        radius = 0.5 * float(extent)
        omin, odim = b.core()[:2]
        cropped = self.cropped = (omin, odim) != (list(b.minp), list(b.dims)) or a.core()[2] is not None
        if self.ratio >= 1:
            step = int(self.ratio)
            if cropped:
                vmin, vdim = ops.lattice_volume_box(omin, odim, step, ops.lattice_reach(a.voxel, radius, dev))
            else:
                vmin, vdim = ops.lattice_volume_box(b.minp, b.dims, step, ops.lattice_reach(a.voxel, radius, dev), a.minp, a.dims)
            res = (vmin, vdim, None)
        else:
            lo = [omin[k] for k in range(3)]
            hi = [omin[k] + odim[k] - 1 for k in range(3)]
            if cropped:
                launches, vlo, vhi = [], [1 << 30] * 3, [-(1 << 30)] * 3
            else:
                launches, vlo, vhi = [], list(a.minp), [a.minp[k] + a.dims[k] - 1 for k in range(3)]
            for pz in (0, 1):
                for py in (0, 1):
                    for px in (0, 1):
                        ph = (px, py, pz)
                        bmin = [-((ph[k] - lo[k]) // 2) for k in range(3)]
                        bmax = [(hi[k] - ph[k]) // 2 for k in range(3)]
                        bdim = [bmax[k] - bmin[k] + 1 for k in range(3)]
                        if min(bdim) <= 0:
                            continue
                        shift = [ph[k] * b.voxel[k] for k in range(3)]
                        m, d = ops.lattice_volume_box(bmin, bdim, 1, ops.lattice_reach(a.voxel, radius, dev, shift))
                        vlo = [min(vlo[k], m[k]) for k in range(3)]
                        vhi = [max(vhi[k], m[k] + d[k] - 1) for k in range(3)]
                        launches.append((ph, bmin, bdim, shift))
            vdim = [vhi[k] - vlo[k] + 1 for k in range(3)]
            parts = [dict(out_phase=ph, rel_shift=shift, base_min=bmin, base_dims=bdim) for ph, bmin, bdim, shift in launches]
            res = (vlo, vdim, parts)
        self._plan = (key, res)
        return res

    def volume_cells(self, ops, extent, dev):
        vdim = self.plan(ops, extent, dev)[1]
        return int(vdim[0]) * int(vdim[1]) * int(vdim[2])

    def conv(self, ops, kernel, inp_features, n_out, extent, **kw):
        a, b = self.inp, self.out
        vmin, vdim, parts = self.plan(ops, extent, inp_features.device)
        if self.cropped:
            omin, odim = b.core()[:2]
            vol, table, tmin = a.volume_in(inp_features, vmin, vdim), b.table_in(omin, odim), omin
            fill = min(1.0, a.gpos.shape[0] / float(max(vdim[0] * vdim[1] * vdim[2], 1)))
        else:
            vol, table, tmin = a.volume(inp_features, vmin, vdim), b.table(), b.minp
            fill = a.gpos.shape[0] / float(a.dims[0] * a.dims[1] * a.dims[2])
        if parts is None:
            return ops.lattice_conv(kernel, vol, vmin, table, tmin, n_out, a.voxel, extent, inp_step=int(self.ratio),
                                    fill=fill, **kw)
        return ops.lattice_conv(kernel, vol, vmin, table, tmin, n_out, a.voxel, extent, inp_step=1, out_stride=2,
                                parts=parts, fill=fill, **kw)

    def strays(self):
        _, _, idx, pos, valid = self.out.core()
        return None if idx is None else (idx, pos, valid)


def pair(inp_positions, out_positions, extent=None):
    if not enabled():
        return None
    a, b = lookup(inp_positions), lookup(out_positions)
    if a is None or b is None or a.family != b.family:
        return None
    if extent is not None:
        if a.max_abs is None or b.max_abs is None or max(a.max_abs, b.max_abs) > MAX_X_OVER_EXTENT * float(extent):
            return None
    if all(a.voxel[k] == 2.0 * b.voxel[k] for k in range(3)):
        return LatticePair(a, b, 0.5)
    step = round(b.voxel[0] / a.voxel[0])
    if step < 1 or any(b.voxel[k] != step * a.voxel[k] for k in range(3)):
        return None
    return LatticePair(a, b, int(step))
```

dmcf_amd/ops.py:

```python
import collections
import os
import ctypes

import threading

import numpy as np
import torch

from . import _lib

class NeighborCapacityExceeded(RuntimeError):
    """A search enqueued with estimated buffer sizes produced more pairs than the buffers hold."""


class NeighborSearchResult:

    def __init__(self, index_buf, row_splits, dist_buf, total=None, redo=None):
        self._index_buf, self._dist_buf = index_buf, dist_buf
        self.neighbors_row_splits = row_splits
        self._total = total
        self._redo = redo

    def raw(self):
        return self._index_buf, self.neighbors_row_splits, self._dist_buf

    def release(self):
        if self._index_buf is not None:
            self._capacity = self._index_buf.shape[0]
        self._index_buf = self._dist_buf = None
        self._redo = None

    @property
    def total_ref(self):
        return self.neighbors_row_splits[-1]

    @property
    def capacity(self):
        return self._index_buf.shape[0] if self._index_buf is not None else self._capacity

    def resolve(self):
        if self._total is None:
            total = int(self.neighbors_row_splits[-1].item())
            if total > self._index_buf.shape[0]:
                self._index_buf, self._dist_buf = self._redo(pair_capacity(total))
            self._total = total
        return self._total

    def overflowed(self, total):
        return self._total is None and total > self.capacity

    @property
    def neighbors_index(self):
        return self._index_buf[:self.resolve()]

    @property
    def neighbors_distance(self):
        n = self.resolve()
        return self._dist_buf[:n] if self._dist_buf.shape[0] >= n else self._dist_buf

    def __iter__(self):
        return iter((self.neighbors_index, self.neighbors_row_splits, self.neighbors_distance))

    def __getitem__(self, i):
        return tuple(self)[i]

    def __len__(self):
        return 3

class PaddedNeighborList(NeighborSearchResult):

    def __init__(self, index_buf, row_begin, dist_buf, counts, max_count, stride, redo_exact):
        super().__init__(index_buf, row_begin, dist_buf, total=None, redo=None)
        self.row_count = counts
        self.max_count = max_count
        self.stride = int(stride)
        self._redo_exact = redo_exact
        self._compact = None

    @property
    def total_ref(self):
        t = getattr(self, "_total_ref", None)
        if t is None:
            small = self.row_count.shape[0] * self.stride < 2 ** 31
            t = self._total_ref = self.row_count.sum(dtype=torch.int32) if small else self.row_count.sum()
        return t

    def release(self):
        super().release()
        self._redo_exact = None
        self._compact = None

    def overflowed(self, max_count):
        return max_count > self.stride

    def resolve(self):
        if self._compact is None:
            if int(self.max_count.item()) > self.stride:
                self._compact = self._redo_exact()
            else:
                m = self.row_count.shape[0]
                cnt = self.row_count.long()
                rs = torch.zeros(m + 1, dtype=torch.int64, device=cnt.device)
                torch.cumsum(cnt, 0, out=rs[1:])
                total = int(rs[-1].item())
                row = torch.repeat_interleave(torch.arange(m, device=cnt.device), cnt, output_size=total)
                src = row * self.stride + (torch.arange(total, device=cnt.device) - rs[:-1][row])
                dist = self._dist_buf[src] if self._dist_buf.shape[0] else self._dist_buf
                self._compact = NeighborSearchResult(self._index_buf[src], rs, dist, total=total)
        return self._compact

    @property
    def neighbors_index(self):
        return self.resolve().neighbors_index

    @property
    def neighbors_distance(self):
        return self.resolve().neighbors_distance

    @property
    def csr_row_splits(self):
        return self.resolve().neighbors_row_splits

    def __iter__(self):
        c = self.resolve()
        return iter((c.neighbors_index, c.neighbors_row_splits, c.neighbors_distance))


MAPPINGS = {"ball_to_cube_radial": 0, "ball_to_cube_volume_preserving": 1, "identity": 2}
INTERPOLATIONS = {"linear": 0, "linear_border": 1, "nearest_neighbor": 2}
WINDOWS = {None: 0, "explicit": 1, "poly6": 2, "cubic": 3, "linear": 4, "peak": 5, "cubic_grad": 6}

FLAG_ALIGN_CORNERS, FLAG_NORMALIZE, FLAG_SYMMETRIC, FLAG_ACCUMULATE, FLAG_SKIP_SELF, FLAG_FILTER_PACKED = 1, 2, 4, 8, 16, 32


class LaunchTimer:

    def __init__(self):
        self.records = []

    def begin(self):
        ev = torch.cuda.Event(enable_timing=True)
        ev.record(torch.cuda.current_stream())
        return ev

    def end(self, kind, meta, start):
        ev = torch.cuda.Event(enable_timing=True)
        ev.record(torch.cuda.current_stream())
        self.records.append((kind, meta, start, ev))

    def results(self):
        out = []
        for k, m, s, e in self.records:
            m = {a: (int(b.item()) if isinstance(b, torch.Tensor) else b) for a, b in m.items()}
            out.append((k, m, s.elapsed_time(e)))
        return out


timer = None


_raw_stream = getattr(torch._C, "_cuda_getCurrentRawStream", None)


def _stream():
    if _raw_stream is not None:
        return ctypes.c_void_p(_raw_stream(torch.cuda.current_device()))
    return ctypes.c_void_p(torch.cuda.current_stream().cuda_stream)


def _dev_f32(t, name, cols=None):
    if not isinstance(t, torch.Tensor):
        raise TypeError(f"{name} must be a torch tensor")
    if not t.is_cuda:
        raise _lib.DmcfError(f"{name} is on {t.device}: the DMCF hot path runs on the GPU only (no CPU fallback)")
    if t.dtype != torch.float32:
        raise TypeError(f"{name} must be float32, got {t.dtype}")
    if cols is not None and (t.dim() != 2 or t.shape[1] != cols):
        raise ValueError(f"{name} must have shape [n,{cols}], got {tuple(t.shape)}")
    t = t.contiguous()
    if t.data_ptr() % 16:
        t = t.clone()
    return t


def _ptr(t):
    return None if t is None else ctypes.c_void_p(t.data_ptr())


class SpatialHashTable:

    def __init__(self, points, radius, workspace, n_queries_capacity):
        self.points = points
        self.radius = float(radius)
        self.workspace = workspace
        self.n_queries_capacity = n_queries_capacity


def build_spatial_hash_table(points, radius, n_queries=None, **_ignored):
    L = _lib.lib()
    points = _dev_f32(points, "points", 3)
    n = points.shape[0]
    m = n if n_queries is None else int(n_queries)
    nbytes = L.dmcf_frs_workspace_bytes(n, m)
    ws = torch.empty(nbytes, dtype=torch.uint8, device=points.device)
    t0 = timer.begin() if timer is not None else None
    _lib.check(L.dmcf_frs_build(_ptr(points), n, float(radius), _ptr(ws), nbytes, _stream()), "dmcf_frs_build")
    if timer is not None:
        timer.end("frs_build", dict(n_points=n), t0)
    return SpatialHashTable(points, radius, ws, m)


def reserve_device_memory(gib, device=None):
    dev = torch.device("cuda", torch.cuda.current_device()) if device is None else torch.device(device)
    before = torch.cuda.memory_stats(dev).get("num_device_alloc", 0)
    try:
        block = torch.empty(int(gib * (1 << 30)), dtype=torch.uint8, device=dev)
    except torch.cuda.OutOfMemoryError:
        return -1.0
    del block
    return float(gib) if torch.cuda.memory_stats(dev).get("num_device_alloc", 0) > before else 0.0


def pair_capacity(total):
    x = int(total) + int(total) // 8 + 65536
    return _size_class(x)


def _size_class(x):
    x = max(int(x), 1)
    if x >= 1 << 27:
        g = 1 << 28
    else:
        g = max(1 << 16, 1 << max(x.bit_length() - 4, 0))
    return (x + g - 1) // g * g


FRS_IGNORE_QUERY_POINT, FRS_OPEN3D_CORNER_VOXELS, FRS_OPEN3D_VOXEL_WALK = 1, 2, 4

SEARCH_SETS = {"distance": 0, "open3d": FRS_OPEN3D_VOXEL_WALK, "open3d_corners": FRS_OPEN3D_CORNER_VOXELS}


_CONSTS = {}


def const_tensor(values, dtype, device):
    key = (tuple(float(v) for v in values), dtype, str(device))
    t = _CONSTS.get(key)
    if t is None:
        if len(_CONSTS) > 256:
            _CONSTS.clear()
        t = _CONSTS[key] = torch.tensor(list(values), dtype=dtype, device=device)
    return t


def search_set():
    if "DMCF_FRS_BRUTE_FORCE_SET" in os.environ:
        raise ValueError("DMCF_FRS_BRUTE_FORCE_SET is gone: use DMCF_FRS_SET=distance (what it selected) | open3d | open3d_corners")
    name = os.environ.get("DMCF_FRS_SET", "distance")
    if name not in SEARCH_SETS:
        raise ValueError(f"DMCF_FRS_SET={name!r}: expected one of {sorted(SEARCH_SETS)}")
    return name


def frs_flags(ignore_query_point):
    return (FRS_IGNORE_QUERY_POINT if ignore_query_point else 0) | SEARCH_SETS[search_set()]


def fixed_radius_search(points, queries, radius, ignore_query_point=False, return_distances=True,
                        hash_table=None, capacity_hint=None, row_stride=None, max_count=None):
    L = _lib.lib()
    points = _dev_f32(points, "points", 3)
    queries = _dev_f32(queries, "queries", 3)
    radius = float(radius)
    if not radius > 0:
        raise ValueError("radius must be positive")
    n, m = points.shape[0], queries.shape[0]
    if hash_table is None or hash_table.n_queries_capacity < m or hash_table.points.data_ptr() != points.data_ptr() \
            or hash_table.radius != radius:
        hash_table = build_spatial_hash_table(points, radius, n_queries=m)
    ws = hash_table.workspace
    nbytes = L.dmcf_frs_workspace_bytes(n, hash_table.n_queries_capacity)
    flags = frs_flags(ignore_query_point)
    dev = points.device
    row_splits = torch.empty(m + 1, dtype=torch.int64, device=dev)
    if row_stride is not None:
# ... 149 lines not shown
        twin = getattr(self, "_index_only", None)
        if twin is None:
            twin = self._index_only = RadiusSearch(self.metric, self.ignore_query_point, False, False)
        return twin


def per_point_extents(extent, n_out):
    if not isinstance(extent, torch.Tensor) or extent.numel() == 1:
        return None
    if extent.dim() == 2 and extent.shape[1] == 3:
        raise NotImplementedError("anisotropic extents [n, 3] are not implemented")
    if tuple(extent.shape) not in ((n_out,), (n_out, 1)):
        raise ValueError(f"per-point extents must have shape [{n_out}] or [{n_out}, 1], got {tuple(extent.shape)}")
    return extent.reshape(n_out)


def _empty(t):
    return t is None or (isinstance(t, torch.Tensor) and t.numel() == 0)


def _extent_operands(extent, n_out):
    ext = per_point_extents(extent, n_out)
    if ext is None:
        return None, extent
    ext = _dev_f32(ext, "extents")
    if n_out > 0 and not bool((torch.isfinite(ext) & (ext > 0)).all()):
        raise ValueError("per-point extents must be finite and positive")
    return ext, 1.0


def _kernel_name(fn, *args, size=96, what=None):
    name = ctypes.create_string_buffer(size)
    rc = fn(*args, name, size)
    if what is not None:
        _lib.check(rc, what)
    return name.value


def _cconv_args(filters, out_positions, extent, inp_positions, inp_features, neighbors_index, neighbors_row_splits, *,
                neighbors_value=None, window=None, window_fac=1.0, inp_importance=None, align_corners=True,
                coordinate_mapping="ball_to_cube_volume_preserving", interpolation="linear", normalize=False, symmetric=False,
                sym_axis=2, bias=None, out=None, accumulate=False, neighbors_row_count=None, filter_tile_mask=0,
                skip_self=False, row_length_hint=0):
    filters = _dev_f32(filters, "filters")
    if filters.dim() != 5:
        raise ValueError("filters must have shape [D,H,W,Cin,Cout]")
    out_positions = _dev_f32(out_positions, "out_positions", 3)
    inp_positions = _dev_f32(inp_positions, "inp_positions", 3)
    cin, cout = filters.shape[3], filters.shape[4]
    if inp_features is not None:
        inp_features = _dev_f32(inp_features, "inp_features", cin)
        if inp_features.shape[0] != inp_positions.shape[0]:
            raise ValueError("inp_features and inp_positions disagree on the number of points")
    n_out = out_positions.shape[0]
    if neighbors_index.dtype != torch.int32 or neighbors_row_splits.dtype != torch.int64:
        raise TypeError("neighbors_index must be int32 and neighbors_row_splits int64")
    if neighbors_row_splits.shape[0] != n_out + 1:
        raise ValueError("neighbors_row_splits must have n_out+1 entries")
    if window not in WINDOWS:
        raise NotImplementedError(f"window {window!r}")
    if window is not None:
        if _empty(neighbors_value):
            if window == "explicit" and neighbors_index.numel() > 0:
                raise ValueError("explicit window but no per-neighbour values")
            neighbors_value = None
        else:
            neighbors_value = _dev_f32(neighbors_value, "neighbors_value")
            if neighbors_value.shape[0] != neighbors_index.shape[0]:
                raise ValueError("neighbors_value and neighbors_index disagree on the number of pairs")
    inp_importance = None if _empty(inp_importance) else _dev_f32(inp_importance, "inp_importance")
    if bias is not None:
        bias = _dev_f32(bias, "bias")
    neighbors_index = neighbors_index.contiguous()
    neighbors_row_splits = neighbors_row_splits.contiguous()
    a = _lib.CconvArgs()
    a.filters = filters.data_ptr()
    for d in range(5):
        a.filter_dims[d] = filters.shape[d]
    a.sym_axis = int(sym_axis)
    a.out_positions = out_positions.data_ptr()
    a.n_out = n_out
    a.inp_positions = inp_positions.data_ptr()
    a.n_inp = inp_positions.shape[0]
    a.inp_features = None if inp_features is None else inp_features.data_ptr()
    a.inp_importance = None if inp_importance is None else inp_importance.data_ptr()
    a.neighbors_index = neighbors_index.data_ptr()
    a.neighbors_row_splits = neighbors_row_splits.data_ptr()
    a.neighbors_value = None if window is None or neighbors_value is None else neighbors_value.data_ptr()
    a.extent = float(extent)
    a.window_fac = float(window_fac)
    a.window = WINDOWS[window]
    a.coordinate_mapping = MAPPINGS[coordinate_mapping]
    a.interpolation = INTERPOLATIONS[interpolation]
    a.flags = ((FLAG_ALIGN_CORNERS if align_corners else 0) | (FLAG_NORMALIZE if normalize else 0) |
               (FLAG_SYMMETRIC if symmetric else 0) | (FLAG_ACCUMULATE if accumulate else 0) | (FLAG_SKIP_SELF if skip_self else 0))
    a.bias = None if bias is None else bias.data_ptr()
    a.out = None if out is None else out.data_ptr()
    a.n_pairs = neighbors_index.shape[0]
    a.neighbors_row_count = None
    a.filter_tile_mask = int(filter_tile_mask) & 0xffffffff
    a.row_length_hint = int(row_length_hint)
    if neighbors_row_count is not None:
        if neighbors_row_count.dtype != torch.int32 or neighbors_row_count.shape[0] != n_out:
            raise TypeError("neighbors_row_count must be int32 [n_out]")
        neighbors_row_count = neighbors_row_count.contiguous()
        a.neighbors_row_count = neighbors_row_count.data_ptr()
    keep = (neighbors_row_count, filters, out_positions, inp_positions, inp_features, inp_importance, neighbors_index, neighbors_row_splits,
            neighbors_value, bias, out)
    return a, keep


_STENCILS = {}


def lattice_offsets(voxel, radius, device, shift=(0.0, 0.0, 0.0)):
    return _stencil(voxel, radius, device, shift)[0]


def lattice_reach(voxel, radius, device, shift=(0.0, 0.0, 0.0)):
    return list(_stencil(voxel, radius, device, shift)[1])


def _stencil(voxel, radius, device, shift):
    key = (tuple(float(v) for v in voxel), float(radius), tuple(float(v) for v in shift), str(device))
    st = _STENCILS.get(key)
    if st is None:
        v, sh = np.asarray(voxel, np.float32), np.asarray(shift, np.float32)
        reach = [int(np.floor((radius + abs(float(c))) / float(x))) + 1 if x > 0 else 0 for x, c in zip(v, sh)]
        ax = [np.arange(-r, r + 1, dtype=np.int32) for r in reach]
        dz, dy, dx = np.meshgrid(ax[2], ax[1], ax[0], indexing="ij")
        x, y, z = dx.astype(np.float32) * v[0] - sh[0], dy.astype(np.float32) * v[1] - sh[1], dz.astype(np.float32) * v[2] - sh[2]
        d2 = (x * x + y * y) + z * z
        keep = d2 <= np.float32(radius) * np.float32(radius)
        off = np.stack([dx[keep], dy[keep], dz[keep], np.zeros(int(keep.sum()), np.int32)], axis=1).astype(np.int32)
        rch = [int(np.abs(off[:, k]).max()) if off.shape[0] else 0 for k in range(3)]
        st = (torch.from_numpy(np.ascontiguousarray(off)).to(device), rch)
        _STENCILS[key] = st
    return st


def lattice_volume_box(base_min, base_dims, inp_step, reach, points_min=None, points_dims=None):
    lo, hi = [], []
    for k in range(3):
        ext = (int(base_dims[k]) + 15) // 16 * 16 if k == 0 else int(base_dims[k])
        l = int(base_min[k]) * inp_step - int(reach[k])
        h = (int(base_min[k]) + ext - 1) * inp_step + int(reach[k])
        if points_min is not None:
            l, h = min(l, int(points_min[k])), max(h, int(points_min[k]) + int(points_dims[k]) - 1)
        lo.append(l)
        hi.append(h)
    return lo, [hi[k] - lo[k] + 1 for k in range(3)]


def _lattice_args(filters, inp_volume, inp_min, out_table, out_min, n_out, voxel, extent, *, inp_step=1, out_stride=1,
                  out_phase=(0, 0, 0), rel_shift=(0.0, 0.0, 0.0), base_min=None, base_dims=None, window="poly6", window_fac=1.0,
                  align_corners=True, coordinate_mapping="ball_to_cube_volume_preserving", interpolation="linear", bias=None,
                  out=None, accumulate=False, parts=None):
    if inp_volume.dim() != 4 or inp_volume.shape[3] != filters.shape[3] or not inp_volume.is_contiguous() or not out_table.is_contiguous():
        raise ValueError("inp_volume must be a contiguous [dz, dy, dx, Cin] tensor, out_table a contiguous [dz, dy, dx] one")
    if parts is None:
        parts = [dict(out_phase=out_phase, rel_shift=rel_shift, base_min=base_min, base_dims=base_dims)]
    arr = (_lib.LatticeConvArgs * len(parts))()
    keep, n_off = [], 0
    for a, pt in zip(arr, parts):
        ph, sh, bmin, bdims = pt["out_phase"], pt["rel_shift"], pt["base_min"], pt["base_dims"]
        offsets, reach = _stencil(voxel, 0.5 * float(extent), filters.device, sh)
        if bmin is None:
            bmin, bdims = out_min, [int(out_table.shape[2 - k]) for k in range(3)]
        a.filters = _ptr(filters)
        for k in range(5):
            a.filter_dims[k] = int(filters.shape[k])
        a.inp_volume, a.out_table = _ptr(inp_volume), _ptr(out_table)
        for k in range(3):
            a.inp_min[k], a.inp_dims[k] = int(inp_min[k]), int(inp_volume.shape[2 - k])
            a.out_min[k], a.out_dims[k] = int(out_min[k]), int(out_table.shape[2 - k])
            a.out_phase[k], a.base_min[k], a.base_dims[k] = int(ph[k]), int(bmin[k]), int(bdims[k])
            a.rel_shift[k], a.voxel[k], a.reach[k] = float(sh[k]), float(voxel[k]), reach[k]
        a.n_out, a.inp_step, a.out_stride = int(n_out), int(inp_step), int(out_stride)
        a.offsets, a.n_offsets = _ptr(offsets), int(offsets.shape[0])
        a.extent, a.window_fac = float(extent), float(window_fac)
        a.window = WINDOWS[window]
        a.coordinate_mapping, a.interpolation = MAPPINGS[coordinate_mapping], INTERPOLATIONS[interpolation]
        a.flags = (FLAG_ALIGN_CORNERS if align_corners else 0) | (FLAG_ACCUMULATE if accumulate else 0)
        a.bias = _ptr(bias) if bias is not None else None
        a.out = _ptr(out)
        keep.append(offsets)
        n_off += int(offsets.shape[0])
    return arr, keep, n_off


def lattice_conv(filters, inp_volume, inp_min, out_table, out_min, n_out, voxel, extent, inp_step=1, out_stride=1,
                 out_phase=(0, 0, 0), rel_shift=(0.0, 0.0, 0.0), base_min=None, base_dims=None, window="poly6",
                 window_fac=1.0, align_corners=True, coordinate_mapping="ball_to_cube_volume_preserving",
                 interpolation="linear", bias=None, out=None, accumulate=False, fill=1.0, n_out_launch=None, parts=None):
    if torch.is_grad_enabled() and any(t is not None and t.requires_grad for t in (filters, inp_volume, bias)):
        if out is not None or accumulate:
            raise ValueError("lattice_conv: out / accumulate cannot be recorded for autograd")
        geo = dict(inp_min=inp_min, out_table=out_table, out_min=out_min, n_out=n_out, voxel=voxel, extent=extent,
                   inp_step=inp_step, out_stride=out_stride, out_phase=out_phase, rel_shift=rel_shift, base_min=base_min,
                   base_dims=base_dims, window=window, window_fac=window_fac, align_corners=align_corners,
                   coordinate_mapping=coordinate_mapping, interpolation=interpolation, parts=parts)
        return LatticeConvFunction.apply(filters, inp_volume, bias, geo, dict(fill=fill, n_out_launch=n_out_launch))
    L = _lib.lib()
    dev = filters.device
    cin, cout = filters.shape[3], filters.shape[4]
    if out is None:
        if accumulate:
            raise ValueError("accumulate=True needs an out tensor")
        out = torch.zeros((n_out, cout), dtype=torch.float32, device=dev)
    filters = filters.contiguous()
    arr, keep, n_off = _lattice_args(filters, inp_volume, inp_min, out_table, out_min, n_out, voxel, extent, inp_step=inp_step,
                                     out_stride=out_stride, out_phase=out_phase, rel_shift=rel_shift, base_min=base_min,
                                     base_dims=base_dims, window=window, window_fac=window_fac, align_corners=align_corners,
                                     coordinate_mapping=coordinate_mapping, interpolation=interpolation, bias=bias, out=out,
                                     accumulate=accumulate, parts=parts)
    if len(arr) == 1:
        nbytes = L.dmcf_lattice_conv_workspace_bytes(arr)
    else:
        nbytes = L.dmcf_lattice_conv_batch_workspace_bytes(arr, len(arr))
    ws = torch.empty(nbytes, dtype=torch.uint8, device=dev)
    t0 = timer.begin() if timer is not None else None
    if len(arr) == 1:
        _lib.check(L.dmcf_lattice_conv_forward(arr, _ptr(ws), nbytes, _stream()), "dmcf_lattice_conv_forward")
    else:
        _lib.check(L.dmcf_lattice_conv_forward_batch(arr, len(arr), _ptr(ws), nbytes, _stream()), "dmcf_lattice_conv_forward_batch")
    if timer is not None:
        no = int(n_out if n_out_launch is None else n_out_launch)
        timer.end("cconv", dict(pairs=0, pairs_equiv=int(no * (n_off / len(arr)) * float(fill)), n_out=no, cin=int(cin),
                                cout=int(cout), K=int(filters.shape[0] * filters.shape[1] * filters.shape[2]), symmetric=False,
                                lattice=True, kernel="lat_conv_kernel", n_offsets=int(n_off), parts=len(arr),
                                volume_bytes=int(inp_volume.numel()) * 4, table_bytes=int(out_table.numel()) * 4,
                                accumulate=bool(accumulate)), t0)
    return out


def lattice_conv_backward(filters, inp_volume, inp_min, out_table, out_min, n_out, voxel, extent, grad_out, inp_step=1,
                          out_stride=1, out_phase=(0, 0, 0), rel_shift=(0.0, 0.0, 0.0), base_min=None, base_dims=None,
                          window="poly6", window_fac=1.0, align_corners=True,
                          coordinate_mapping="ball_to_cube_volume_preserving", interpolation="linear", parts=None,
                          need_volume=True, need_filters=True):
    L = _lib.lib()
    filters = _dev_f32(filters, "filters")
    dev = filters.device
    grad_out = _dev_f32(grad_out, "grad_out", filters.shape[4])
    if grad_out.shape[0] != n_out:
        raise ValueError("grad_out must be [n_out, Cout]")
    if not need_volume and not need_filters:
        return None, None
    arr, keep, _ = _lattice_args(filters, inp_volume, inp_min, out_table, out_min, n_out, voxel, extent, inp_step=inp_step,
                                 out_stride=out_stride, out_phase=out_phase, rel_shift=rel_shift, base_min=base_min,
                                 base_dims=base_dims, window=window, window_fac=window_fac, align_corners=align_corners,
                                 coordinate_mapping=coordinate_mapping, interpolation=interpolation, out=grad_out, parts=parts)
    gv = torch.empty_like(inp_volume) if need_volume else None
    gw = torch.empty_like(filters) if need_filters else None
    nbytes = int(L.dmcf_lattice_conv_backward_workspace_bytes(arr, len(arr)))
    ws = torch.empty(nbytes, dtype=torch.uint8, device=dev)
    t0 = timer.begin() if timer is not None else None
    _lib.check(L.dmcf_lattice_conv_backward(arr, len(arr), _ptr(grad_out), _ptr(gv), _ptr(gw), _ptr(ws), nbytes, _stream()),
               "dmcf_lattice_conv_backward")
    if timer is not None:
        timer.end("cconv_backward", dict(n_out=int(n_out), cin=int(filters.shape[3]), cout=int(filters.shape[4]),
                                         filters=bool(need_filters), features=bool(need_volume), lattice=True, parts=len(arr),
                                         kernel="lat_bwd_filter;lat_bwd_input"), t0)
    del keep
    return gv, gw


class LatticeConvFunction(torch.autograd.Function):

    @staticmethod
    def forward(ctx, filters, inp_volume, bias, geo, info):
        ctx.geo = geo
        ctx.has_bias = bias is not None
        ctx.save_for_backward(filters, inp_volume)
        return lattice_conv(filters, inp_volume, bias=bias, **geo, **info)

    @staticmethod
    def backward(ctx, grad_out):
        filters, inp_volume = ctx.saved_tensors
        need_w, need_v = ctx.needs_input_grad[0], ctx.needs_input_grad[1]
        need_b = ctx.has_bias and ctx.needs_input_grad[2]
        grad_out = grad_out.contiguous()
        gv, gw = lattice_conv_backward(filters.detach(), inp_volume.detach(), grad_out=grad_out, need_volume=need_v,
                                       need_filters=need_w, **ctx.geo)
        gb = None
        if need_b:
            n_out = int(ctx.geo["n_out"])
            rows = ctx.geo["out_table"].reshape(-1).long()
            hit = torch.zeros(n_out + 1, dtype=grad_out.dtype, device=grad_out.device)
            hit[torch.where(rows >= 0, rows, torch.full_like(rows, n_out))] = 1.0
            gb = (grad_out * hit[:n_out, None]).sum(0)
        return gw, gv, gb, None, None


def block_diagonal_tile_mask(blocks):
    mask = 0
    for c0, c1, o0, o1 in blocks:
        if c1 > 32 or o1 > 64:
            return 0
        for q in range(c0 // 4, (c1 + 3) // 4):
            for n in range(o0 // 16, (o1 + 15) // 16):
                mask |= 1 << (4 * q + n)
    return mask


def cconv_forward(filters, out_positions, extent, inp_positions, inp_features, neighbors_index,
                  neighbors_row_splits, neighbors_value=None, window=None, window_fac=1.0, inp_importance=None,
                  align_corners=True, coordinate_mapping="ball_to_cube_volume_preserving", interpolation="linear",
                  normalize=False, symmetric=False, sym_axis=2, bias=None, out=None, accumulate=False,
                  n_pairs_ref=None, neighbors_row_count=None, filter_tile_mask=0, skip_self=False, name_only=False,
                  row_length_hint=0, packed_cache=None, record_per_point_extents=False):
    if not name_only and torch.is_grad_enabled() and (
            (isinstance(filters, torch.Tensor) and filters.requires_grad) or
            (isinstance(inp_features, torch.Tensor) and inp_features.requires_grad) or
            (isinstance(bias, torch.Tensor) and bias.requires_grad)):
        if out is not None or accumulate:
            raise ValueError("out= / accumulate=True cannot be recorded by autograd: use the returned tensor")
        ext = per_point_extents(extent, out_positions.shape[0])
        if ext is not None and not record_per_point_extents:
            raise NotImplementedError("recording CConv with per-point extents is opt-in: pass record_per_point_extents=True "
                                      "(the backward is dmcf_cconv_backward_extents; the extents get no gradient)")
        geo = dict(out_positions=out_positions, extent=float(extent) if ext is None else ext.detach(), inp_positions=inp_positions,
                   neighbors_index=neighbors_index, neighbors_row_splits=neighbors_row_splits, neighbors_value=neighbors_value,
                   window=window, window_fac=window_fac, inp_importance=inp_importance, align_corners=align_corners,
                   coordinate_mapping=coordinate_mapping, interpolation=interpolation, normalize=normalize, symmetric=symmetric,
                   sym_axis=sym_axis, neighbors_row_count=neighbors_row_count, skip_self=skip_self)
        res = CconvFunction.apply(filters, inp_features, geo, dict(filter_tile_mask=filter_tile_mask, row_length_hint=row_length_hint,
                                                                   n_pairs_ref=n_pairs_ref, packed_cache=packed_cache))
        if bias is not None:
            res = res + bias
        return res
    L = _lib.lib()
    n_out, cout = out_positions.shape[0], filters.shape[4]
    ext, extent = _extent_operands(extent, n_out)
    if out is None:
        if accumulate:
            raise ValueError("accumulate=True needs an out tensor")
        out = torch.empty((n_out, cout), dtype=torch.float32, device=filters.device)
    elif out.shape != (n_out, cout) or out.dtype != torch.float32 or not out.is_contiguous():
        raise ValueError("out has the wrong shape / dtype / layout")
    if inp_positions.shape[0] == 0 or n_out == 0:
        b = 0.0 if bias is None else bias.to(torch.float32)
        if accumulate:
            out += b
        else:
            out[:] = b
        return out
    a, keep = _cconv_args(filters, out_positions, extent, inp_positions, inp_features, neighbors_index, neighbors_row_splits,
                          neighbors_value=neighbors_value, window=window, window_fac=window_fac, inp_importance=inp_importance,
                          align_corners=align_corners, coordinate_mapping=coordinate_mapping, interpolation=interpolation,
                          normalize=normalize, symmetric=symmetric, sym_axis=sym_axis, bias=bias, out=out, accumulate=accumulate,
                          neighbors_row_count=neighbors_row_count, filter_tile_mask=filter_tile_mask, skip_self=skip_self,
                          row_length_hint=row_length_hint)
    kernel_name = L.dmcf_cconv_kernel_name if ext is None else L.dmcf_cconv_extents_kernel_name
    if name_only:
        return _kernel_name(kernel_name, ctypes.byref(a), what="dmcf_cconv_kernel_name").decode()
    nbytes = L.dmcf_cconv_workspace_bytes(ctypes.byref(a))
    ws = None
    if packed_cache is not None and ext is None:
        key = (filters._version, tuple(filters.shape), bool(symmetric), int(sym_axis),
               _kernel_name(L.dmcf_cconv_kernel_name, ctypes.byref(a)), str(filters.device))
        ws = packed_cache.get("ws")
        if packed_cache.get("src") is filters and packed_cache.get("key") == key and ws is not None and ws.numel() >= nbytes:
            a.flags |= FLAG_FILTER_PACKED
        else:
            ws = torch.empty(nbytes + nbytes // 4, dtype=torch.uint8, device=filters.device)
            packed_cache["key"], packed_cache["ws"], packed_cache["src"] = key, ws, filters
        nbytes = ws.numel()
    if ws is None:
        ws = torch.empty(nbytes, dtype=torch.uint8, device=filters.device)
    t0 = timer.begin() if timer is not None else None
    if ext is None:
        _lib.check(L.dmcf_cconv_forward(ctypes.byref(a), _ptr(ws), nbytes, _stream()), "dmcf_cconv_forward")
# ... 1266 lines not shown
```

dmcf_amd/utils/convolutions.py:

```python
import math
import os
import threading

import numpy as np
import torch

from .. import ops
from .tools.losses import WindowFunction

__all__ = ["ContinuousConv", "neighbor_cache"]

SCATTER_OUT_CHANNELS = (4,)
SCATTER_MIN_INPUTS = 4096
SCATTER_MAX_LATTICE_CELLS = 1 << 16
SMALL_LIST_ENTRIES = 1 << 21


class _NeighborCache:

    def __init__(self):
        self.depth = 0
        self.hints = {}
        self.caps = {}
        self.totals = {}
# ... 228 lines not shown
            _CACHE.use_hints = bool(self.estimate) and os.environ.get("DMCF_NO_ESTIMATE") != "1"
            _CACHE._get().select(self.key)
            self.outer = True
        else:
            self.outer = False
        return _CACHE.__enter__()

    def __exit__(self, *exc):
        try:
            return _CACHE.__exit__(*exc)
        finally:
            if self.outer:
                _CACHE.use_hints = self.prev


def neighbor_cache(estimate=False, key=None):
    return _CacheScope(estimate, key)


def pairs_ref(nns):
    return nns.total_ref if ops.timer is not None else None


def _scatter_guard(vals):
    if any(vals):
        raise RuntimeError("dmcf_cconv_scatter_forward dropped pairs: a block's box did not hold an output it reaches (plan / positions mismatch)")
    return False


def _hint_key(frs, points, queries, radius):
    def size_class(n):
        return int(round(2.0 * math.log2(max(int(n), 1))))
    return (float(radius), size_class(points.shape[0]), size_class(queries.shape[0]), bool(frs.ignore_query_point),
            bool(frs.return_distances))


class _HintView:

    def __init__(self, hints):
        self._hints = hints

    def __iter__(self):
        return iter(list(self._hints.values()))

    def __len__(self):
        return len(self._hints)

    def clear(self):
        self._hints.clear()


def neighbor_hints():
    return _HintView(_CACHE.hints)


def row_stride(longest):
    longest = int(longest)
    x = longest + max(longest // 4, min(longest, 64)) + 8
    g = max(8, 1 << max(x.bit_length() - 4, 0))
    return (x + g - 1) // g * g


def _init_tensor(name, shape, device):
    if callable(name):
        return name(shape).to(device)
    if name == "uniform":
        return torch.empty(shape, device=device).uniform_(-0.05, 0.05)
    if name == "zeros":
        return torch.zeros(shape, device=device)
    if name == "glorot_uniform":
        fan_in, fan_out = shape[-2] * int(np.prod(shape[:-2])), shape[-1] * int(np.prod(shape[:-2]))
        limit = math.sqrt(6.0 / (fan_in + fan_out))
        return torch.empty(shape, device=device).uniform_(-limit, limit)
    raise NotImplementedError(f"initializer {name!r}")


_ACTIVATIONS = {None: None, "linear": None, "relu": torch.relu, "tanh": torch.tanh}


def _rank1_extents(extents, out_positions):
    return (isinstance(extents, torch.Tensor) and extents.dim() == 1
            and (extents.numel() > 1 or extents.numel() == out_positions.shape[0]))


class PlainAttributes:

    def __setattr__(self, name, value):
        d = self.__dict__
        if (isinstance(value, (torch.nn.Parameter, torch.nn.Module)) or "_parameters" not in d or name in d["_parameters"]
                or name in d["_buffers"] or name in d["_modules"] or hasattr(type(self), name)):
            super().__setattr__(name, value)
        else:
            d[name] = value


class ContinuousConv(PlainAttributes, torch.nn.Module):

    def __init__(self, filters, kernel_size, activation=None, use_bias=True, kernel_initializer="uniform",
                 bias_initializer="zeros", kernel_regularizer=None, bias_regularizer=None, align_corners=True,
                 coordinate_mapping="ball_to_cube_radial", interpolation="linear", normalize=True,
                 radius_search_ignore_query_points=False, radius_search_metric="L2", offset=None,
                 window_function=None, use_dense_layer_for_center=False,
                 dense_kernel_initializer="glorot_uniform", dense_kernel_regularizer=None, in_channels=None,
                 symmetric=False, sym_axis=2, circular=False, name=None, trainable=True, device=None,
                 record_per_point_extents=False, record_lattice_form=False, **kwargs):
        super().__init__()
        self.layer_name = name
        self.record_per_point_extents = bool(record_per_point_extents)
        self.record_lattice_form = bool(record_lattice_form)
        self.filters = filters
        self.kernel_size = [int(k) for k in kernel_size]
        if activation not in _ACTIVATIONS and not callable(activation):
            raise NotImplementedError(f"activation {activation!r}")
        self.activation = _ACTIVATIONS.get(activation, activation) if not callable(activation) else activation
        self.use_bias = use_bias
        self.kernel_initializer = kernel_initializer
        self.bias_initializer = bias_initializer
        self.align_corners = align_corners
        if coordinate_mapping not in ops.MAPPINGS:
            raise ValueError(f"coordinate_mapping {coordinate_mapping!r}")
        if interpolation not in ops.INTERPOLATIONS:
            raise ValueError(f"interpolation {interpolation!r}")
        self.coordinate_mapping = coordinate_mapping
        self.interpolation = interpolation
        self.normalize = normalize
        self.radius_search_ignore_query_points = radius_search_ignore_query_points
        self.radius_search_metric = radius_search_metric
        self.dense_kernel_initializer = dense_kernel_initializer
        self.symmetric = symmetric
        self.sym_axis = sym_axis
        self.circular = circular
        if offset is not None and any(float(o) != 0.0 for o in torch.as_tensor(offset).reshape(-1)):
            raise NotImplementedError("non-zero offset (never used by DMCF, convolutions.py:200-201)")
        self.offset = torch.zeros(3)
        self.window_function = window_function
        self.fixed_radius_search = ops.FixedRadiusSearch(
            metric=self.radius_search_metric, ignore_query_point=self.radius_search_ignore_query_points,
            return_distances=self.window_function is not None)
        self.radius_search = ops.RadiusSearch(
            metric=self.radius_search_metric, ignore_query_point=self.radius_search_ignore_query_points,
            return_distances=self.window_function is not None, normalize_distances=self.window_function is not None)
        self.use_dense_layer_for_center = use_dense_layer_for_center
        self.dense = None
        self.in_channels = None
        self.kernel = None
        self.bias = None
        self._device = device
        self.nns = None
        self._direct_kernel = None
        self.row_length_hint = 0
        self.accumulate_into = None
        self.extra_bias = None
        self._packed = {}

    def invalidate_packed(self):
        self._packed.clear()

    def _load_from_state_dict(self, *args, **kwargs):
        self._packed.clear()
        return super()._load_from_state_dict(*args, **kwargs)

    def build(self, in_channels, device=None):
        self._packed.clear()
        device = device or self._device or "cuda"
        self.in_channels = int(in_channels)
        if self.circular:
            kshape = (math.ceil(max(self.kernel_size) / 2), self.in_channels, self.filters)
        elif self.symmetric:
            sh = list(self.kernel_size)
            assert sh[self.sym_axis] % 2 == 0
            sh[self.sym_axis] = sh[self.sym_axis] // 2
            kshape = (*sh, self.in_channels, self.filters)
        else:
            kshape = (*self.kernel_size, self.in_channels, self.filters)
        self.kernel = torch.nn.Parameter(_init_tensor(self.kernel_initializer, kshape, device), requires_grad=False)
        if self.use_bias:
            self.bias = torch.nn.Parameter(_init_tensor(self.bias_initializer, (self.filters,), device),
                                           requires_grad=False)
        if self.use_dense_layer_for_center:
            w = _init_tensor(self.dense_kernel_initializer, (self.in_channels, self.filters), device)
            self.dense = torch.nn.Parameter(w, requires_grad=False)

    def _expanded_kernel(self):
        ks = self.kernel_size
        zr, yr, xr = torch.meshgrid(*[torch.arange(k, device=self.kernel.device) for k in ks], indexing="ij")
        size_xyz = torch.tensor(ks[::-1], dtype=torch.float32, device=self.kernel.device)
        gp = torch.stack([xr, yr, zr], dim=-1).to(torch.float32) - size_xyz / 2.0 + 0.5
        mask = (gp * 2.0) / size_xyz
        idx = torch.floor(gp.abs()).max(dim=-1).values.to(torch.int64)
        kernel = self.kernel[idx]
        if self.symmetric:
            kernel = kernel * mask.unsqueeze(-2)
        return kernel

    def forward(self, inp_features, inp_positions, out_positions, extents, inp_importance=None,
                fixed_radius_search_hash_table=None, user_neighbors_index=None, user_neighbors_row_splits=None,
                user_neighbors_importance=None):
        if self.kernel is None:
            with torch.no_grad():
                self.build(inp_features.shape[-1], inp_features.device)
        if self.recording(inp_features):
            return self._forward_train(inp_features, inp_positions, out_positions, extents, inp_importance,
                                       fixed_radius_search_hash_table, user_neighbors_index, user_neighbors_row_splits,
                                       user_neighbors_importance)
        return self._forward_infer(inp_features, inp_positions, out_positions, extents, inp_importance,
                                   fixed_radius_search_hash_table, user_neighbors_index, user_neighbors_row_splits,
                                   user_neighbors_importance)

    def recording(self, inp_features=None):
        if not torch.is_grad_enabled():
            return False
        if isinstance(inp_features, torch.Tensor) and inp_features.requires_grad:
            return True
        return any(w is not None and w.requires_grad for w in (self.kernel, self.bias, self.dense))

    def _forward_train(self, inp_features, inp_positions, out_positions, extents, inp_importance, hash_table,
                       user_neighbors_index, user_neighbors_row_splits, user_neighbors_importance):
        d = self.__dict__
        acc, extra_bias = self.accumulate_into, self.extra_bias
        d["accumulate_into"] = d["extra_bias"] = None
        window, window_fac, neighbors_value = None, 1.0, None
        row_count = None
        rank1 = _rank1_extents(extents, out_positions)
        if rank1 and not self.record_per_point_extents:
            raise NotImplementedError("ContinuousConv with per-point extents (rank 1) records only when built with "
                                      "record_per_point_extents=True; without it the training path takes a scalar extent only")
        if rank1:
            with torch.no_grad():
                extent = extents.detach()
                neighbors_index, neighbors_row_splits, window, window_fac, neighbors_value = self._extents_lists(
                    inp_positions, out_positions, extent, user_neighbors_index, user_neighbors_row_splits, user_neighbors_importance)
        elif isinstance(extents, torch.Tensor):
            if extents.dim() > 0 and extents.numel() != 1:
                raise NotImplementedError("extents must be a scalar or of rank 1, [n_out] (convolutions.py:352-372)")
            extent = float(extents)
        else:
            extent = float(np.float32(extents))
        lat = None
        if self.record_lattice_form and not rank1 and (user_neighbors_index is None or user_neighbors_row_splits is None):
            lat = self._lattice_form(inp_features, inp_positions, out_positions, inp_importance, hash_table, extent)
            if lat is not None and (lat.cropped or lat.ratio not in (1, 2, 0.5)):
                lat = None
        if lat is not None:
            d["nns"] = None
            d["_n_out_last"] = out_positions.shape[0]
            d["_pairs_last"] = 0
            d["_conv_values"] = None
            out_features = lat.conv(ops, self.kernel, inp_features, out_positions.shape[0], extent,
                                    window=self.window_function.name, window_fac=self.window_function.fac,
                                    align_corners=self.align_corners, coordinate_mapping=self.coordinate_mapping,
                                    interpolation=self.interpolation)
            return self._train_epilogue(out_features, inp_features, acc, extra_bias)
        if rank1:
            pass
        elif user_neighbors_index is not None and user_neighbors_row_splits is not None:
            neighbors_index, neighbors_row_splits = user_neighbors_index, user_neighbors_row_splits
            if user_neighbors_importance is not None and user_neighbors_importance.numel() > 0:
                window, neighbors_value = "explicit", user_neighbors_importance
        else:
            radius = float(np.float32(0.5) * np.float32(extent))
            with torch.no_grad():
                if hash_table is not None:
                    d["nns"] = self.fixed_radius_search(inp_positions, out_positions, radius, hash_table=hash_table)
                else:
                    d["nns"] = self.fixed_radius_search(inp_positions, out_positions, radius)
                neighbors_index, neighbors_row_splits, raw_dist = self.nns.raw()
                row_count = getattr(self.nns, "row_count", None)
                if self.window_function is not None:
                    if isinstance(self.window_function, WindowFunction):
                        window, window_fac = self.window_function.name, self.window_function.fac
                        neighbors_value = raw_dist
                    else:
                        q = self.nns.neighbors_distance / (np.float32(radius) * np.float32(radius))
                        neighbors_index = self.nns.neighbors_index
                        if row_count is not None:
                            neighbors_row_splits, row_count = self.nns.csr_row_splits, None
                        window, neighbors_value = "explicit", self.window_function(q).to(torch.float32)
        d["_n_out_last"] = out_positions.shape[0]
        d["_pairs_last"] = neighbors_index.shape[0]
        kernel, symmetric = self._conv_kernel()
        d["_conv_values"] = None
        out_features = ops.cconv_forward(
            kernel, out_positions, extent, inp_positions, inp_features, neighbors_index, neighbors_row_splits,
            neighbors_value=neighbors_value, window=window, window_fac=window_fac, inp_importance=inp_importance,
            align_corners=self.align_corners, coordinate_mapping=self.coordinate_mapping,
            interpolation=self.interpolation, normalize=self.normalize, symmetric=symmetric, sym_axis=self.sym_axis,
            neighbors_row_count=row_count, row_length_hint=self.row_length_hint,
            packed_cache=self._packed if (kernel is self.kernel and os.environ.get("DMCF_CACHE_PACKED_FILTERS", "1") != "0")
            else None, **({"record_per_point_extents": True} if rank1 else {}))
        return self._train_epilogue(out_features, inp_features, acc, extra_bias)

    def _train_epilogue(self, out_features, inp_features, acc, extra_bias):
        if self.use_bias and not self.use_dense_layer_for_center:
            out_features = out_features + self.bias
        self.__dict__["_conv_output"] = None
        out_features = self._finish(out_features, inp_features, extra_bias if acc is None else None)
        if acc is not None:
            out_features = acc + out_features
            if extra_bias is not None:
                out_features = out_features + extra_bias
        return out_features

    @torch.no_grad()
    def _forward_infer(self, inp_features, inp_positions, out_positions, extents, inp_importance=None,
                       fixed_radius_search_hash_table=None, user_neighbors_index=None, user_neighbors_row_splits=None,
                       user_neighbors_importance=None):
        acc, extra_bias = self.accumulate_into, self.extra_bias
        d = self.__dict__
        d["accumulate_into"] = d["extra_bias"] = None
        if acc is not None and (self.use_dense_layer_for_center or self.activation is not None or not acc.is_contiguous()
                                or tuple(acc.shape) != (out_positions.shape[0], self.filters) or acc.dtype != torch.float32):
            acc.add_(self.forward(inp_features, inp_positions, out_positions, extents, inp_importance,
                                  fixed_radius_search_hash_table, user_neighbors_index, user_neighbors_row_splits,
                                  user_neighbors_importance))
            return acc if extra_bias is None else acc.add_(extra_bias)
        if _rank1_extents(extents, out_positions):
            return self._forward_extents(inp_features, inp_positions, out_positions, extents, inp_importance, user_neighbors_index,
                                         user_neighbors_row_splits, user_neighbors_importance, acc, extra_bias)
        if isinstance(extents, torch.Tensor):
            if extents.dim() > 0 and extents.numel() != 1:
                raise NotImplementedError("extents must be a scalar or of rank 1, [n_out] (convolutions.py:352-372)")
            extent = float(extents)
        else:
            extent = float(np.float32(extents))
        window, window_fac, neighbors_value, n_pairs_ref, row_count = None, 1.0, None, None, None
        skip_self = False
        if user_neighbors_index is not None and user_neighbors_row_splits is not None:
            neighbors_index, neighbors_row_splits = user_neighbors_index, user_neighbors_row_splits
            if user_neighbors_importance is not None and user_neighbors_importance.numel() > 0:
                window, neighbors_value = "explicit", user_neighbors_importance
        else:
            lat = self._lattice_form(inp_features, inp_positions, out_positions, inp_importance,
                                     fixed_radius_search_hash_table, extent)
            if lat is not None:
                d["nns"] = None
                fuse_bias = self.use_bias and not self.use_dense_layer_for_center
                d["_n_out_last"] = out_positions.shape[0]
                d["_pairs_last"] = 0
                out_features = lat.conv(
                    ops, self.kernel, inp_features, out_positions.shape[0], extent,
                    window=self.window_function.name, window_fac=self.window_function.fac,
                    align_corners=self.align_corners, coordinate_mapping=self.coordinate_mapping,
                    interpolation=self.interpolation, bias=self._epilogue_bias(fuse_bias, extra_bias),
                    out=acc, accumulate=acc is not None)
                stray = lat.strays()
                if stray is not None:
                    idx_s, pos_s, valid = stray
                    radius = float(np.float32(0.5) * np.float32(extent))
                    nns = _CACHE.search(self.fixed_radius_search, inp_positions, pos_s, radius, distances=False)
                    ni, nrs, raw_dist = nns.raw()
                    res = ops.cconv_forward(
                        self.kernel, pos_s, extent, inp_positions, inp_features, ni, nrs, neighbors_value=raw_dist,
                        window=self.window_function.name, window_fac=self.window_function.fac, align_corners=self.align_corners,
                        coordinate_mapping=self.coordinate_mapping, interpolation=self.interpolation,
                        bias=self._epilogue_bias(fuse_bias, extra_bias), n_pairs_ref=pairs_ref(nns),
                        neighbors_row_count=getattr(nns, "row_count", None), row_length_hint=1)
                    if valid is not None:
                        res = res * valid
                    out_features.index_add_(0, idx_s, res)
                d["_conv_values"], d["_conv_output"] = None, (None if _CACHE.depth > 0 else out_features)
                return self._finish(out_features, inp_features, extra_bias if self.use_dense_layer_for_center else None)
            radius = float(np.float32(0.5) * np.float32(extent))
            sct = self._scatter_form(inp_features, inp_positions, out_positions, inp_importance, fixed_radius_search_hash_table,
                                     radius)
            if sct is not None:
                voxel, m = sct
                tl = _CACHE.search(self.fixed_radius_search, out_positions, inp_positions, radius, distances=False)
                t_idx, t_rb, _ = tl.raw()
                d["nns"] = None
                d["_n_out_last"] = out_positions.shape[0]
                d["_pairs_last"] = tl
                fuse_bias = self.use_bias and not self.use_dense_layer_for_center
                flag = _CACHE._max_count_slot(inp_positions.device) if _CACHE.depth > 0 else torch.zeros(1, dtype=torch.int32, device=inp_positions.device)
                out_features = ops.cconv_scatter_forward(
                    self.kernel, out_positions, extent, inp_positions, inp_features, t_idx, t_rb, getattr(tl, "row_count", None),
                    _CACHE.scatter_plan(inp_positions, out_positions, voxel, radius, m), window=self.window_function.name,
                    window_fac=self.window_function.fac, bias=self._epilogue_bias(fuse_bias, extra_bias), out=acc,
                    accumulate=acc is not None, n_pairs_ref=pairs_ref(tl), error_flag=flag)
                _CACHE.report(flag, _scatter_guard)
                d["_conv_values"], d["_conv_output"] = None, (None if _CACHE.depth > 0 else out_features)
                return self._finish(out_features, inp_features, extra_bias if self.use_dense_layer_for_center else None)
            if fixed_radius_search_hash_table is not None:
                d["nns"] = self.fixed_radius_search(inp_positions, out_positions, radius,
                                                    hash_table=fixed_radius_search_hash_table)
            else:
                shared = None
                if self._shares_list():
                    shared = _CACHE.with_query_points(self.fixed_radius_search, inp_positions, out_positions, radius)
                skip_self = shared is not None
                d["nns"] = shared if skip_self else _CACHE.search(
                    self.fixed_radius_search, inp_positions, out_positions, radius,
                    distances=not isinstance(self.window_function, WindowFunction))
            neighbors_index, neighbors_row_splits, raw_dist = self.nns.raw()
            row_count = getattr(self.nns, "row_count", None)
            n_pairs_ref = pairs_ref(self.nns)
            if self.window_function is not None:
                if isinstance(self.window_function, WindowFunction):
                    window, window_fac = self.window_function.name, self.window_function.fac
                    neighbors_value = raw_dist
                else:
                    q = self.nns.neighbors_distance / (np.float32(radius) * np.float32(radius))
                    neighbors_index = self.nns.neighbors_index
                    if row_count is not None:
                        neighbors_row_splits, row_count = self.nns.csr_row_splits, None
                    window, neighbors_value = "explicit", self.window_function(q).to(torch.float32)
        d["_n_out_last"] = out_positions.shape[0]
        d["_pairs_last"] = self.nns if (n_pairs_ref is None and getattr(self, "nns", None) is not None and user_neighbors_index is None) \
            else (n_pairs_ref if n_pairs_ref is not None else neighbors_index.shape[0])

        kernel, symmetric = self._conv_kernel()
        in_step = _CACHE.depth > 0
        d["_conv_values"] = {
            "filters": kernel, "out_positions": out_positions, "extents": extent, "offset": self.offset,
            "inp_positions": inp_positions, "inp_features": None if in_step else inp_features,
            "inp_importance": inp_importance,
            "neighbors_index": None if in_step else neighbors_index, "neighbors_row_splits": neighbors_row_splits,
            "neighbors_importance": None if in_step else neighbors_value, "align_corners": self.align_corners,
            "coordinate_mapping": self.coordinate_mapping, "interpolation": self.interpolation,
            "normalize": self.normalize,
        }
        fuse_bias = self.use_bias and not self.use_dense_layer_for_center
        out_features = ops.cconv_forward(
            kernel, out_positions, extent, inp_positions, inp_features, neighbors_index, neighbors_row_splits,
            neighbors_value=neighbors_value, window=window, window_fac=window_fac, inp_importance=inp_importance,
            align_corners=self.align_corners, coordinate_mapping=self.coordinate_mapping,
            interpolation=self.interpolation, normalize=self.normalize, symmetric=symmetric, sym_axis=self.sym_axis,
            bias=self._epilogue_bias(fuse_bias, extra_bias), n_pairs_ref=n_pairs_ref,
            neighbors_row_count=row_count, skip_self=skip_self, row_length_hint=self.row_length_hint,
            out=acc, accumulate=acc is not None,
            packed_cache=self._packed if (kernel is self.kernel and os.environ.get("DMCF_CACHE_PACKED_FILTERS", "1") != "0")
            else None)
        if self._direct_kernel is None and in_step and self.radius_search_ignore_query_points:
            self._direct_kernel = ops.cconv_forward(
                kernel, out_positions, extent, inp_positions, inp_features, neighbors_index, neighbors_row_splits,
                neighbors_value=neighbors_value, window=window, window_fac=window_fac, inp_importance=inp_importance,
                align_corners=self.align_corners, coordinate_mapping=self.coordinate_mapping,
                interpolation=self.interpolation, normalize=self.normalize, symmetric=symmetric, sym_axis=self.sym_axis,
                neighbors_row_count=row_count, name_only=True).startswith("cconv_direct_kernel")
            if self._shares_list() and user_neighbors_index is None and fixed_radius_search_hash_table is None:
                _CACHE.with_query_points(self.fixed_radius_search, inp_positions, out_positions,
                                         float(np.float32(0.5) * np.float32(extent)))
        d["_conv_output"] = None if in_step else out_features
        return self._finish(out_features, inp_features, extra_bias if self.use_dense_layer_for_center else None)

    def _conv_kernel(self):
        kernel, symmetric = self.kernel, self.symmetric
        if self.circular:
            if self.symmetric:
                raise NotImplementedError("circular + symmetric kernels (filters must be 3 in the reference; "
                                          "no shipped config uses circular: True)")
            kernel = self._expanded_kernel()
            symmetric = False
        if symmetric and self.normalize:
            raise NotImplementedError("symmetric=True with normalize=True (DMCF always uses normalize=False, "
                                      "models/pbf_model.py:203)")
        return kernel, symmetric

    def _extents_lists(self, inp_positions, out_positions, extents, user_neighbors_index, user_neighbors_row_splits,
                       user_neighbors_importance):
        n_out = out_positions.shape[0]
        if extents.shape[0] != n_out:
            raise ValueError(f"extents of rank 1 must hold one value per output point ({n_out}), got {extents.shape[0]}")
        window, window_fac, neighbors_value = None, 1.0, None
        if user_neighbors_index is not None and user_neighbors_row_splits is not None:
            neighbors_index, neighbors_row_splits = user_neighbors_index, user_neighbors_row_splits
            if user_neighbors_importance is not None and user_neighbors_importance.numel() > 0:
                window, neighbors_value = "explicit", user_neighbors_importance
        else:
            radii = 0.5 * extents
            named = isinstance(self.window_function, WindowFunction)
            search = self.radius_search.index_only() if named else self.radius_search
            self.__dict__["nns"] = search(inp_positions, out_positions, radii)
            neighbors_index, neighbors_row_splits, dist = self.nns
            if self.window_function is not None:
                if named:
                    window, window_fac = self.window_function.name, self.window_function.fac
                else:
                    window, neighbors_value = "explicit", self.window_function(dist).to(torch.float32)
        return neighbors_index, neighbors_row_splits, window, window_fac, neighbors_value

    def _forward_extents(self, inp_features, inp_positions, out_positions, extents, inp_importance, user_neighbors_index,
                         user_neighbors_row_splits, user_neighbors_importance, acc, extra_bias):
        d = self.__dict__
        n_out = out_positions.shape[0]
        neighbors_index, neighbors_row_splits, window, window_fac, neighbors_value = self._extents_lists(
            inp_positions, out_positions, extents, user_neighbors_index, user_neighbors_row_splits, user_neighbors_importance)
        d["_n_out_last"] = n_out
        d["_pairs_last"] = neighbors_index.shape[0]
        kernel, symmetric = self._conv_kernel()
        in_step = _CACHE.depth > 0
        d["_conv_values"] = {
            "filters": kernel, "out_positions": out_positions, "extents": extents.reshape(n_out, 1), "offset": self.offset,
            "inp_positions": inp_positions, "inp_features": None if in_step else inp_features,
            "inp_importance": inp_importance,
            "neighbors_index": None if in_step else neighbors_index, "neighbors_row_splits": neighbors_row_splits,
            "neighbors_importance": None if in_step else neighbors_value, "align_corners": self.align_corners,
            "coordinate_mapping": self.coordinate_mapping, "interpolation": self.interpolation,
# ... 162 lines not shown
```

include/dmcf_hip.h:

```cpp
#ifndef DMCF_HIP_H_
#define DMCF_HIP_H_

#include <stddef.h>
#include <stdint.h>

#ifdef __cplusplus
extern "C" {
#endif

#define DMCF_OK 0
#define DMCF_EINVAL (-1)
#define DMCF_EWORKSPACE (-2)
#define DMCF_ELAUNCH (-3)
#define DMCF_EUNSUPPORTED (-4)

typedef void* dmcf_stream_t;

int dmcf_version(void);
const char* dmcf_error_string(int code);
int dmcf_last_hip_error(void);

#define DMCF_FRS_IGNORE_QUERY_POINT 1
#define DMCF_FRS_OPEN3D_CORNER_VOXELS 2
#define DMCF_FRS_OPEN3D_VOXEL_WALK 4
// ... 32 lines not shown
                             int64_t pair_capacity, dmcf_stream_t stream);

enum dmcf_mapping {
    DMCF_MAP_BALL_TO_CUBE_RADIAL = 0,
    DMCF_MAP_BALL_TO_CUBE_VOLUME_PRESERVING = 1,
    DMCF_MAP_IDENTITY = 2
};
enum dmcf_interpolation { DMCF_INTERP_LINEAR = 0, DMCF_INTERP_LINEAR_BORDER = 1, DMCF_INTERP_NEAREST = 2 };
enum dmcf_window {
    DMCF_WINDOW_NONE = 0,
    DMCF_WINDOW_EXPLICIT = 1,
    DMCF_WINDOW_POLY6 = 2,
    DMCF_WINDOW_CUBIC = 3,
    DMCF_WINDOW_LINEAR = 4,
    DMCF_WINDOW_PEAK = 5,
    DMCF_WINDOW_CUBIC_GRAD = 6
};
#define DMCF_FLAG_ALIGN_CORNERS 1
#define DMCF_FLAG_NORMALIZE 2
#define DMCF_FLAG_SYMMETRIC 4
#define DMCF_FLAG_ACCUMULATE 8
#define DMCF_FLAG_FILTER_PACKED 32
#define DMCF_FLAG_SKIP_SELF 16

typedef struct dmcf_cconv_args {
    const float* filters;
    int32_t filter_dims[5];
    int32_t sym_axis;
    const float* out_positions;
    int64_t n_out;
    const float* inp_positions;
    int64_t n_inp;
    const float* inp_features;
    const float* inp_importance;
    const int32_t* neighbors_index;
    const int64_t* neighbors_row_splits;
    const float* neighbors_value;
    float extent;
    float window_fac;
    int32_t window;
    int32_t coordinate_mapping;
    int32_t interpolation;
    int32_t flags;
    const float* bias;
    float* out;
    int64_t n_pairs;
    const int32_t* neighbors_row_count;
    uint32_t filter_tile_mask;
    int32_t row_length_hint;
} dmcf_cconv_args;

size_t dmcf_cconv_workspace_bytes(const dmcf_cconv_args* args);

int dmcf_cconv_forward(const dmcf_cconv_args* args, void* workspace, size_t workspace_bytes,
                       dmcf_stream_t stream);
int dmcf_cconv_kernel_name(const dmcf_cconv_args* args, char* name, size_t name_bytes);

int dmcf_cconv_forward_extents(const dmcf_cconv_args* args, const float* out_extents, void* workspace,
                               size_t workspace_bytes, dmcf_stream_t stream);
int dmcf_cconv_extents_kernel_name(const dmcf_cconv_args* args, char* name, size_t name_bytes);

size_t dmcf_invert_neighbors_list_workspace_bytes(int64_t n_pairs);
int dmcf_invert_neighbors_list(int64_t n_inp, const int32_t* neighbors_index, const int64_t* neighbors_row_splits,
                               const int32_t* neighbors_row_count, int64_t n_out, int64_t n_pairs, const float* values,
                               int32_t* inv_index, int64_t* inv_row_splits, int32_t* inv_pair, float* inv_values,
                               void* workspace, size_t workspace_bytes, dmcf_stream_t stream);

#define DMCF_BWD_ACCUMULATE 1
typedef struct dmcf_cconv_backward_args {
    uint32_t struct_size;
    int32_t flags;
    const float* grad_out;
    const int32_t* inv_index;
    const int32_t* inv_pair;
    const int64_t* inv_row_splits;
    int64_t inv_n_rows;
    int64_t inv_n_pairs;
    float* grad_filters;
    float* grad_inp_features;
} dmcf_cconv_backward_args;

size_t dmcf_cconv_backward_workspace_bytes(const dmcf_cconv_args* fwd, const dmcf_cconv_backward_args* bwd);
int dmcf_cconv_backward(const dmcf_cconv_args* fwd, const dmcf_cconv_backward_args* bwd, void* workspace,
                        size_t workspace_bytes, dmcf_stream_t stream);
int dmcf_cconv_backward_kernel_names(const dmcf_cconv_args* fwd, const dmcf_cconv_backward_args* bwd, char* names,
                                     size_t name_bytes);

int dmcf_cconv_backward_extents(const dmcf_cconv_args* fwd, const dmcf_cconv_backward_args* bwd, const float* out_extents,
                                void* workspace, size_t workspace_bytes, dmcf_stream_t stream);
int dmcf_cconv_backward_extents_kernel_names(const dmcf_cconv_args* fwd, const dmcf_cconv_backward_args* bwd, char* names,
                                             size_t name_bytes);

size_t dmcf_cconv_scatter_plan_bytes(int64_t n_inp);
int dmcf_cconv_scatter_plan(const float* inp_positions, int64_t n_inp, const float* out_positions, int64_t n_out, float voxel,
                            float extent, int32_t block_cells, void* plan, size_t plan_bytes, dmcf_stream_t stream);

typedef struct dmcf_cconv_scatter_args {
    const float* filters;
    int32_t filter_dims[5];
    const float* out_positions;
    int64_t n_out;
    const float* inp_positions;
    int64_t n_inp;
    const float* inp_features;
    const int32_t* t_index;
    const int64_t* t_row_begin;
    const int32_t* t_row_count;
    int64_t t_capacity;
    const void* plan;
    int32_t block_cells;
    int32_t reach;
    float extent;
    float window_fac;
    int32_t window;
    int32_t flags;
    const float* bias;
    float* out;
    int32_t* error_flag;
} dmcf_cconv_scatter_args;

size_t dmcf_cconv_scatter_workspace_bytes(const dmcf_cconv_scatter_args* args);
int dmcf_cconv_scatter_forward(const dmcf_cconv_scatter_args* args, void* workspace, size_t workspace_bytes,
                               dmcf_stream_t stream);

typedef struct dmcf_lattice_conv_args {
    const float* filters;
    int32_t filter_dims[5];
    const float* inp_volume;
    int32_t inp_min[3];
    int32_t inp_dims[3];
    const int32_t* out_table;
    int32_t out_min[3];
    int32_t out_dims[3];
    int64_t n_out;
    int32_t inp_step;
    int32_t out_stride;
    int32_t out_phase[3];
    int32_t base_min[3], base_dims[3];
    float rel_shift[3];
    float voxel[3];
    const int32_t* offsets;
    int64_t n_offsets;
    int32_t reach[3];
    float extent;
    float window_fac;
    int32_t window;
    int32_t coordinate_mapping;
    int32_t interpolation;
    int32_t flags;
    const float* bias;
    float* out;
} dmcf_lattice_conv_args;

size_t dmcf_lattice_conv_workspace_bytes(const dmcf_lattice_conv_args* args);
int dmcf_lattice_conv_forward(const dmcf_lattice_conv_args* args, void* workspace, size_t workspace_bytes,
                              dmcf_stream_t stream);
size_t dmcf_lattice_conv_batch_workspace_bytes(const dmcf_lattice_conv_args* parts, int32_t n_parts);
int dmcf_lattice_conv_forward_batch(const dmcf_lattice_conv_args* parts, int32_t n_parts, void* workspace,
                                    size_t workspace_bytes, dmcf_stream_t stream);

size_t dmcf_lattice_conv_backward_workspace_bytes(const dmcf_lattice_conv_args* parts, int32_t n_parts);
int dmcf_lattice_conv_backward(const dmcf_lattice_conv_args* parts, int32_t n_parts, const float* grad_out,
                               float* grad_volume, float* grad_filters, void* workspace, size_t workspace_bytes,
                               dmcf_stream_t stream);

int dmcf_reduce_subarrays_sum(const float* values, const int64_t* row_splits, int64_t n_rows, float* out,
                              dmcf_stream_t stream);

int dmcf_dense_forward(const float* x, int64_t n, int32_t k, const float* W, int32_t m, const float* bias,
                       const float* residual, float* out, dmcf_stream_t stream);

size_t dmcf_points_aabb_workspace_bytes(void);
int dmcf_points_aabb(const float* points, int64_t n, float* out, void* workspace, size_t workspace_bytes,
                     dmcf_stream_t stream);

size_t dmcf_ghost_workspace_bytes(int64_t n, int32_t n_boxes, int32_t n_widths);
int dmcf_ghost_count(const float* points, int64_t n, const float* boxes, int32_t n_boxes, const float* widths2, int32_t n_widths,
                     int64_t* totals, void* workspace, size_t workspace_bytes, dmcf_stream_t stream);
int dmcf_ghost_write(const float* points, int64_t n, const float* boxes, int32_t n_boxes, const float* widths2, int32_t n_widths,
                     int64_t* rows, const int64_t* list_start, const int64_t* list_capacity, void* workspace, size_t workspace_bytes,
                     dmcf_stream_t stream);

size_t dmcf_grid_pos_workspace_bytes(int64_t n_points);
int dmcf_grid_pos_bounds(const float* positions, int64_t n_points, const float* voxel_size, int centralize,
                         const float* center, int pad, float hyst, void* workspace, size_t workspace_bytes,
                         dmcf_stream_t stream);
int dmcf_grid_pos_count(const float* positions, int64_t n_points, const float* voxel_size, int centralize, int pad,
                        float hyst, void* workspace, size_t workspace_bytes, void* cell_table, int64_t table_cells,
                        dmcf_stream_t stream);
int dmcf_grid_pos_write(const float* positions, int64_t n_points, const float* voxel_size, int centralize, int pad,
                        float hyst, void* workspace, size_t workspace_bytes, const void* cell_table, int64_t table_cells,
                        float* out, int64_t out_capacity, dmcf_stream_t stream);

size_t dmcf_fps_workspace_bytes(int64_t n_points);
int dmcf_farthest_point_sample(const float* points, int64_t n_points, int64_t n_samples, void* workspace,
                               size_t workspace_bytes, int32_t* sample_index, dmcf_stream_t stream);
int dmcf_gather_point(const float* inp, const int32_t* index, int64_t n_index, int channels, float* out,
                      dmcf_stream_t stream);

size_t dmcf_nn_distance_workspace_bytes(int64_t b, int64_t n, int64_t m);
int dmcf_nn_distance(const float* xyz1, const float* xyz2, int64_t b, int64_t n, int64_t m, float* dist1, int32_t* idx1,
                     float* dist2, int32_t* idx2, void* workspace, size_t workspace_bytes, dmcf_stream_t stream);
size_t dmcf_approx_match_workspace_bytes(int64_t b, int64_t n, int64_t m);
int dmcf_approx_match(const float* xyz1, const float* xyz2, int64_t b, int64_t n, int64_t m, const int32_t* count1,
                      const int32_t* count2, float* match, void* workspace, size_t workspace_bytes, dmcf_stream_t stream);
size_t dmcf_match_cost_workspace_bytes(int64_t b, int64_t n, int64_t m);
int dmcf_match_cost(const float* xyz1, const float* xyz2, int64_t b, int64_t n, int64_t m, const float* match, float* cost,
                    void* workspace, size_t workspace_bytes, dmcf_stream_t stream);
size_t dmcf_emd_workspace_bytes(int64_t b, int64_t n, int64_t m);
int dmcf_emd(const float* xyz1, const float* xyz2, int64_t b, int64_t n, int64_t m, const int32_t* count1, const int32_t* count2,
             float* cost, void* workspace, size_t workspace_bytes, dmcf_stream_t stream);

size_t dmcf_nn_distance_backward_workspace_bytes(int64_t b, int64_t n, int64_t m);
int dmcf_nn_distance_backward(const float* xyz1, const float* xyz2, int64_t b, int64_t n, int64_t m, const int32_t* idx1,
                              const int32_t* idx2, const float* grad_dist1, const float* grad_dist2, float* grad_xyz1,
                              float* grad_xyz2, void* workspace, size_t workspace_bytes, dmcf_stream_t stream);
size_t dmcf_match_cost_backward_workspace_bytes(int64_t b, int64_t n, int64_t m);
int dmcf_match_cost_backward(const float* xyz1, const float* xyz2, int64_t b, int64_t n, int64_t m, const float* match,
                             const float* grad_cost, float* grad_xyz1, float* grad_xyz2, void* workspace, size_t workspace_bytes,
                             dmcf_stream_t stream);
int dmcf_emd_with_levels(const float* xyz1, const float* xyz2, int64_t b, int64_t n, int64_t m, const int32_t* count1,
                         const int32_t* count2, float* cost, float* levels, void* workspace, size_t workspace_bytes,
                         dmcf_stream_t stream);
size_t dmcf_emd_backward_workspace_bytes(int64_t b, int64_t n, int64_t m);
int dmcf_emd_backward(const float* xyz1, const float* xyz2, int64_t b, int64_t n, int64_t m, const int32_t* count1,
                      const int32_t* count2, const float* levels, const float* grad_cost, float* grad_xyz1, float* grad_xyz2,
                      void* workspace, size_t workspace_bytes, dmcf_stream_t stream);
size_t dmcf_gather_point_backward_workspace_bytes(int64_t n_index, int64_t n_inp);
int dmcf_gather_point_backward(const float* grad_out, const int32_t* index, int64_t n_index, int channels, int64_t n_inp,
                               float* grad_inp, void* workspace, size_t workspace_bytes, dmcf_stream_t stream);

#define DMCF_ND_RELU 1
#define DMCF_ND_W_TRANSPOSED 2
typedef struct dmcf_neighbor_dense_args {
    uint32_t struct_size;
    int32_t flags;
    const float* x;
    int64_t n_in;
    int32_t cin;
    int32_t cout;
    const float* kernel;
    const float* bias;
    const float* residual;
    const float* mask;
    const int32_t* neighbors_index;
    const int64_t* neighbors_row_splits;
    const int32_t* neighbors_row_count;
    int64_t n_out;
    int64_t n_pairs;
    const int64_t* host_row_splits;
    float* out;
    float* record_s;
    float* record_count;
} dmcf_neighbor_dense_args;

int dmcf_neighbor_dense_forward(const dmcf_neighbor_dense_args* args, dmcf_stream_t stream);

typedef struct dmcf_neighbor_dense_backward_args {
    uint32_t struct_size;
    int32_t flags;
    const float* x;
    int64_t n_in;
    int32_t cin;
    int32_t cout;
    const float* kernel;
    const float* grad_out;
    int64_t n_out;
    const float* s;
    const float* count;
    const int32_t* inv_index;
    const int64_t* inv_row_splits;
    int64_t inv_n_pairs;
    float* grad_x;
    float* grad_kernel;
    float* grad_bias;
} dmcf_neighbor_dense_backward_args;

size_t dmcf_neighbor_dense_backward_workspace_bytes(const dmcf_neighbor_dense_backward_args* args);
int dmcf_neighbor_dense_backward(const dmcf_neighbor_dense_backward_args* args, void* workspace, size_t workspace_bytes,
                                 dmcf_stream_t stream);
int dmcf_neighbor_dense_kernel_names(const dmcf_neighbor_dense_args* fwd, const dmcf_neighbor_dense_backward_args* bwd,
                                     char* names, size_t name_bytes);

typedef struct dmcf_adam_tensor {
    float* param;
    const float* grad;
    float* m;
    float* v;
    int64_t n;
} dmcf_adam_tensor;

typedef struct dmcf_adam_args {
    uint32_t struct_size;
    int32_t n_tensors;
    const dmcf_adam_tensor* tensors;
    const dmcf_adam_tensor* device_tensors;
    float lr;
    float beta_1;
    float beta_2;
    float epsilon;
    float beta_1_power;
    float beta_2_power;
    float clip_norm;
    int32_t reserved;
} dmcf_adam_args;

size_t dmcf_adam_step_workspace_bytes(const dmcf_adam_args* args);
int dmcf_adam_step(const dmcf_adam_args* args, void* workspace, size_t workspace_bytes, dmcf_stream_t stream);
int dmcf_adam_step_kernel_names(const dmcf_adam_args* args, char* names, size_t name_bytes);

size_t dmcf_raster_workspace_bytes(int64_t n_points, int64_t n_frames, int64_t frame_stride, int32_t width, int32_t height);
int dmcf_raster_count(const float* xy, int64_t n_points, int64_t n_frames, int64_t frame_stride, float radius, int32_t width,
// ... 28 lines not shown
```

Before: 13.38 million.

## Add parity-split lattice volume, fused lattice build kernel, packed-filter caching, wider row groups

Adds a parity-split (8 sub-volume) layout for stride-2 lattice inputs so strided reads become contiguous. It also adds a fused GPU kernel that builds the occupancy table and scatters features into the volume. Packed lattice filters are cached across calls, keyed on the filter version, so the per-call filter-packing kernel is skipped. A wider 256-row workgroup is chosen when there are enough groups per CU. Together these add more kernel variants, more cache-invalidation logic and more layout branches.

```diff
diff --git a/dmcf_amd/_lib.py b/dmcf_amd/_lib.py
--- a/dmcf_amd/_lib.py
+++ b/dmcf_amd/_lib.py
@@ -133,6 +133,22 @@
     ]
 
 
+class LatticeBuildArgs(ctypes.Structure):
+    _fields_ = [
+        ("positions", ctypes.c_void_p),
+        ("n_points", ctypes.c_int64),
+        ("center", ctypes.c_void_p),
+        ("voxel", ctypes.c_float * 3),
+        ("box_min", ctypes.c_int32 * 3),
+        ("box_dims", ctypes.c_int32 * 3),
+        ("features", ctypes.c_void_p),
+        ("channels", ctypes.c_int32),
+        ("flags", ctypes.c_int32),
+        ("table", ctypes.c_void_p),
+        ("volume", ctypes.c_void_p),
+    ]
+
+
 class CconvScatterArgs(ctypes.Structure):
     _fields_ = [
         ("filters", ctypes.c_void_p),
@@ -214,7 +230,7 @@
     "dmcf_cconv_scatter_plan_bytes", "dmcf_cconv_scatter_plan", "dmcf_cconv_scatter_workspace_bytes", "dmcf_cconv_scatter_forward",
     "dmcf_lattice_conv_workspace_bytes", "dmcf_lattice_conv_forward",
     "dmcf_lattice_conv_batch_workspace_bytes", "dmcf_lattice_conv_forward_batch",
-    "dmcf_lattice_conv_backward_workspace_bytes", "dmcf_lattice_conv_backward",
+    "dmcf_lattice_conv_backward_workspace_bytes", "dmcf_lattice_conv_backward", "dmcf_lattice_build",
     "dmcf_reduce_subarrays_sum", "dmcf_points_aabb_workspace_bytes", "dmcf_points_aabb", "dmcf_dense_forward",
     "dmcf_fps_workspace_bytes", "dmcf_farthest_point_sample", "dmcf_gather_point",
     "dmcf_grid_pos_workspace_bytes", "dmcf_grid_pos_bounds", "dmcf_grid_pos_count", "dmcf_grid_pos_write",
@@ -398,6 +414,8 @@
     L.dmcf_raster_discs.restype = c.c_int
     L.dmcf_raster_discs.argtypes = [c.c_void_p, c.c_int64, c.c_int64, c.c_int64, c.c_float, c.c_uint32, c.c_int32, c.c_int32, c.c_void_p,
                                     c.c_void_p, c.c_size_t, c.c_void_p, c.c_int64, c.c_void_p]
+    L.dmcf_lattice_build.restype = c.c_int
+    L.dmcf_lattice_build.argtypes = [c.POINTER(LatticeBuildArgs), c.c_void_p]
     for q in ("dmcf_nn_distance_backward_workspace_bytes", "dmcf_match_cost_backward_workspace_bytes",
               "dmcf_emd_backward_workspace_bytes"):
         getattr(L, q).restype = c.c_size_t
diff --git a/dmcf_amd/csrc/cconv_lat.hip b/dmcf_amd/csrc/cconv_lat.hip
--- a/dmcf_amd/csrc/cconv_lat.hip
+++ b/dmcf_amd/csrc/cconv_lat.hip
@@ -6,6 +6,7 @@
     const float* Wp;
     const int32_t* stencil;
     int S, KS, NT, cin, cout;
+    int split;
     const float* vol;
     int imin[3], idim[3];
     const int32_t* otab;
@@ -23,16 +24,32 @@
 constexpr int kLatMaxParts = 8;
 constexpr int kLatRowsPerGroup = 128;
 constexpr int kLatCellsPerBlock = 1024;
+constexpr int kLatMinGroupsPerCU = 4;
 struct LatBatch {
     LatParams part[kLatMaxParts];
     int64_t cfirst[kLatMaxParts + 1];
     int n;
+    int rpg;
     uint32_t* blk;
     int64_t* start;
     int64_t* count;
     lat_i32x2* rows;
     int64_t rows_capacity;
 };
+
+__device__ __forceinline__ int lat_rowb_of(const LatParams& p, int ax, int ay, int az) {
+    if (p.split)
+        return (((az - p.imin[2]) * p.idim[1] + (ay - p.imin[1])) * p.idim[0] + (ax - p.imin[0])) * p.cin * 4;
+    const int ix = ax * p.inp_step - p.imin[0], iy = ay * p.inp_step - p.imin[1], iz = az * p.inp_step - p.imin[2];
+    return ((iz * p.idim[1] + iy) * p.idim[0] + ix) * p.cin * 4;
+}
+__device__ __forceinline__ int lat_dof_of(const LatParams& p, int dx, int dy, int dz) {
+    if (p.split) {
+        const int sub = (dz & 1) * 4 + (dy & 1) * 2 + (dx & 1);
+        return (((sub * p.idim[2] + (dz >> 1)) * p.idim[1] + (dy >> 1)) * p.idim[0] + (dx >> 1)) * p.cin * 4;
+    }
+    return ((dz * p.idim[1] + dy) * p.idim[0] + dx) * p.cin * 4;
+}
 
 __device__ __forceinline__ int lat_cell(const LatParams& p, int64_t c, int& rowb) {
     const int64_t tile = c >> 4;
@@ -47,8 +64,7 @@
     if (!(xb * 16 + m < p.adim[0] && (unsigned)ox < (unsigned)p.odim[0] && (unsigned)oy < (unsigned)p.odim[1] &&
           (unsigned)oz < (unsigned)p.odim[2]))
         return -1;
-    const int ix = ax * p.inp_step - p.imin[0], iy = ay * p.inp_step - p.imin[1], iz = az * p.inp_step - p.imin[2];
-    rowb = ((iz * p.idim[1] + iy) * p.idim[0] + ix) * p.cin * 4;
+    rowb = lat_rowb_of(p, ax, ay, az);
     return p.otab[((int64_t)oz * p.odim[1] + oy) * p.odim[0] + ox];
 }
 
@@ -82,7 +98,7 @@
         const int64_t n = (int64_t)b.blk[b.cfirst[i + 1]] - (int64_t)b.blk[b.cfirst[i]];
         b.start[i] = s;
         b.count[i] = n;
-        s += (n + kLatRowsPerGroup - 1) / kLatRowsPerGroup * kLatRowsPerGroup;
+        s += (n + b.rpg - 1) / b.rpg * b.rpg;
     }
     b.start[b.n] = s;
 }
@@ -155,12 +171,10 @@
     }
 }
 
-constexpr int kLatTW = 2;
 constexpr int kLatCH = 32;
 constexpr int kLatG = kLatCH / 4;
-static_assert(kLatRowsPerGroup == 4 * kLatTW * 16, "rows of a workgroup");
-
-template <int NTT, int KST>
+
+template <int NTT, int KST, int kLatTW>
 __device__ __forceinline__ void lat_conv_body(const LatParams& p, const lat_i32x2* __restrict__ rows, const int64_t first, const int64_t end) {
     __shared__ __attribute__((aligned(16))) float Ws[2][kLatCH * KST * NTT * 64];
     const int lane = threadIdx.x & 63, wave = threadIdx.x >> 6;
@@ -174,8 +188,7 @@
     for (int t = 0; t < kLatTW; ++t) {
         const int64_t e = first + ((wave * kLatTW + t) << 4) + m;
         oidx[t] = -1;
-        rowb[t] = (((p.amin[2] * p.inp_step - p.imin[2]) * p.idim[1] + (p.amin[1] * p.inp_step - p.imin[1])) * p.idim[0] +
-                   (p.amin[0] * p.inp_step - p.imin[0])) * p.cin * 4;
+        rowb[t] = lat_rowb_of(p, p.amin[0], p.amin[1], p.amin[2]);
         if (e < end) {
             const lat_i32x2 rw = rows[e];
             rowb[t] = rw.x;
@@ -213,7 +226,7 @@
     for (int s0 = 0, k = 0; s0 < p.S; s0 += kLatCH, ++k) {
         const int ng = min(kLatG, NG - s0 / 4);
         const float* Wc = Ws[k & 1];
-        const int dof = ((dv.z * p.idim[1] + dv.y) * p.idim[0] + dv.x) * p.cin * 4;
+        const int dof = lat_dof_of(p, dv.x, dv.y, dv.z);
         int dofg[kLatG];
 #pragma unroll
         for (int g = 0; g < kLatG; ++g) dofg[g] = __shfl(dof, 4 * g + q, 64);
@@ -273,13 +286,13 @@
     }
 }
 
-template <int NTT, int KST>
+template <int NTT, int KST, int TW>
 __global__ __launch_bounds__(256) void lat_conv_kernel(const LatBatch b) {
-    const int64_t first = (int64_t)blockIdx.x * kLatRowsPerGroup;
+    const int64_t first = (int64_t)blockIdx.x * (64 * TW);
     if (first >= b.start[b.n]) return;
     int i = 0;
     while (i + 1 < b.n && first >= b.start[i + 1]) ++i;
-    lat_conv_body<NTT, KST>(b.part[i], b.rows, first, b.start[i] + b.count[i]);
+    lat_conv_body<NTT, KST, TW>(b.part[i], b.rows, first, b.start[i] + b.count[i]);
 }
 
 static size_t lat_packed_floats(const dmcf_lattice_conv_args* a) {
@@ -297,6 +310,7 @@
     for (int k = 0; k < 3; ++k)
         if (a->inp_dims[k] <= 0 || a->out_dims[k] <= 0 || a->base_dims[k] <= 0 || !(a->voxel[k] >= 0.0f)) return DMCF_EINVAL;
     if (a->flags & (DMCF_FLAG_SYMMETRIC | DMCF_FLAG_NORMALIZE)) return DMCF_EUNSUPPORTED;
+    if ((a->flags & DMCF_FLAG_LATTICE_SPLIT) && a->inp_step != 2) return DMCF_EINVAL;
     if (a->window == DMCF_WINDOW_EXPLICIT) return DMCF_EUNSUPPORTED;
     const int cin = a->filter_dims[3], cout = a->filter_dims[4];
     if ((cin != 4 && cin != 8) || cout > 32) return DMCF_EUNSUPPORTED;
@@ -332,9 +346,17 @@
         const int64_t hi = ((int64_t)a->base_min[k] + ext - 1) * a->inp_step + a->reach[k];
         if (a->reach[k] < 0 || lo < a->inp_min[k] || hi > (int64_t)a->inp_min[k] + a->inp_dims[k] - 1) return DMCF_EINVAL;
     }
-    if ((int64_t)a->inp_dims[0] * a->inp_dims[1] * a->inp_dims[2] * cin > 0x1fffffff) return DMCF_EUNSUPPORTED;
+    p.split = (a->flags & DMCF_FLAG_LATTICE_SPLIT) ? 1 : 0;
+    int64_t vol_cells = (int64_t)a->inp_dims[0] * a->inp_dims[1] * a->inp_dims[2];
+    int hmin[3], hdim[3];
+    for (int k = 0; k < 3; ++k) {
+        hmin[k] = a->inp_min[k] >> 1;
+        hdim[k] = ((a->inp_min[k] + a->inp_dims[k] - 1) >> 1) - hmin[k] + 1;
+    }
+    if (p.split) vol_cells = 8 * (int64_t)hdim[0] * hdim[1] * hdim[2];
+    if (vol_cells * cin > 0x1fffffff) return DMCF_EUNSUPPORTED;
     const CconvParams cp = lat_cconv_params(a);
-    if (a->n_offsets > 0) {
+    if (a->n_offsets > 0 && !(a->flags & DMCF_FLAG_FILTER_PACKED)) {
         const int64_t total = (int64_t)lat_packed_floats(a);
         const unsigned g = (unsigned)((total + 255) / 256);
         hipLaunchKernelGGL(lat_build_filters, dim3(g < 4096u ? g : 4096u), dim3(256), 0, stream, a->filters, packed, a->offsets,
@@ -347,7 +369,7 @@
     p.vol = a->inp_volume;
     p.otab = a->out_table;
     for (int k = 0; k < 3; ++k) {
-        p.imin[k] = a->inp_min[k]; p.idim[k] = a->inp_dims[k];
+        p.imin[k] = p.split ? hmin[k] : a->inp_min[k]; p.idim[k] = p.split ? hdim[k] : a->inp_dims[k];
         p.omin[k] = a->out_min[k]; p.odim[k] = a->out_dims[k];
         p.phase[k] = a->out_phase[k];
         p.amin[k] = a->base_min[k];
@@ -365,10 +387,20 @@
 struct LatLayout {
     size_t off_blk, off_scan, off_tmp, tmp_bytes, off_start, off_rows, total;
     int64_t nblk, rows_capacity;
+    int rpg;
 };
 
-static LatLayout lat_layout(const dmcf_lattice_conv_args* parts, int n_parts) {
+static int lat_pick_rows(const dmcf_lattice_conv_args* parts, int n_parts) {
+    if (parts[0].filter_dims[4] > 16) return kLatRowsPerGroup;
+    const char* e = getenv("DMCF_LAT_ROWS");
+    if (e && *e) return atoi(e) == 2 * kLatRowsPerGroup ? 2 * kLatRowsPerGroup : kLatRowsPerGroup;
+    const int64_t groups = (parts[0].n_out + 2 * kLatRowsPerGroup - 1) / (2 * kLatRowsPerGroup) + n_parts - 1;
+    return groups >= (int64_t)kLatMinGroupsPerCU * device_cu_count() ? 2 * kLatRowsPerGroup : kLatRowsPerGroup;
+}
+
+static LatLayout lat_layout(const dmcf_lattice_conv_args* parts, int n_parts, int rpg = kLatRowsPerGroup) {
     LatLayout L;
+    L.rpg = rpg;
     size_t off = 256;
     L.nblk = 0;
     for (int i = 0; i < n_parts; ++i) {
@@ -381,7 +413,7 @@
     L.tmp_bytes = scan_tmp_bytes(L.nblk + 1);
     L.off_tmp = off;    off += align_up(L.tmp_bytes, 256);
     L.off_start = off;  off += 256;
-    L.rows_capacity = (parts[0].n_out + kLatRowsPerGroup - 1) / kLatRowsPerGroup * kLatRowsPerGroup + (int64_t)kLatRowsPerGroup * n_parts;
+    L.rows_capacity = (parts[0].n_out + rpg - 1) / rpg * rpg + (int64_t)rpg * n_parts;
     L.off_rows = off;   off += align_up((size_t)L.rows_capacity * sizeof(lat_i32x2), 256);
     L.total = off;
     return L;
@@ -423,6 +455,7 @@
     b.count = b.start + kLatMaxParts + 1;
     b.rows = (lat_i32x2*)(ws + L.off_rows);
     b.rows_capacity = L.rows_capacity;
+    b.rpg = L.rpg;
     hipLaunchKernelGGL(lat_rows_count, dim3((unsigned)L.nblk), dim3(256), 0, stream, b);
     const int rc = scan_exclusive_u32(blk_in, (uint32_t*)(ws + L.off_scan), L.nblk + 1, ws + L.off_tmp, L.tmp_bytes, stream);
     if (rc != DMCF_OK) return rc;
@@ -436,20 +469,105 @@
     int rc = lat_check(parts, n_parts);
     if (rc != DMCF_OK) return rc;
     if (parts[0].n_out == 0) return DMCF_OK;
-    const LatLayout L = lat_layout(parts, n_parts);
+    const LatLayout L = lat_layout(parts, n_parts, lat_pick_rows(parts, n_parts));
     LatBatch b;
     rc = lat_rows(parts, n_parts, workspace, workspace_bytes, L.total, stream, b, L);
     if (rc != DMCF_OK) return rc;
-    const dim3 grid((unsigned)(L.rows_capacity / kLatRowsPerGroup)), block(256);
+    const dim3 grid((unsigned)(L.rows_capacity / L.rpg)), block(256);
     const int KS = b.part[0].KS, NT = b.part[0].NT;
-    if (KS == 1 && NT == 1) hipLaunchKernelGGL((lat_conv_kernel<1, 1>), grid, block, 0, stream, b);
-    else if (KS == 1) hipLaunchKernelGGL((lat_conv_kernel<2, 1>), grid, block, 0, stream, b);
-    else if (NT == 1) hipLaunchKernelGGL((lat_conv_kernel<1, 2>), grid, block, 0, stream, b);
-    else hipLaunchKernelGGL((lat_conv_kernel<2, 2>), grid, block, 0, stream, b);
+    const bool wide = L.rpg == 2 * kLatRowsPerGroup;
+    if (KS == 1 && NT == 1 && wide) hipLaunchKernelGGL((lat_conv_kernel<1, 1, 4>), grid, block, 0, stream, b);
+    else if (KS == 1 && NT == 1) hipLaunchKernelGGL((lat_conv_kernel<1, 1, 2>), grid, block, 0, stream, b);
+    else if (KS == 1) hipLaunchKernelGGL((lat_conv_kernel<2, 1, 2>), grid, block, 0, stream, b);
+    else if (NT == 1 && wide) hipLaunchKernelGGL((lat_conv_kernel<1, 2, 4>), grid, block, 0, stream, b);
+    else if (NT == 1) hipLaunchKernelGGL((lat_conv_kernel<1, 2, 2>), grid, block, 0, stream, b);
+    else hipLaunchKernelGGL((lat_conv_kernel<2, 2, 2>), grid, block, 0, stream, b);
     return check_launch();
 }
 
 #include "cconv_lat_bwd.inc"
+
+struct LatBuild {
+    const float* pos;
+    const float* center;
+    float voxel[3];
+    int bmin[3], bdim[3];
+    int hmin[3], hdim[3];
+    int split;
+    const float* feat;
+    int C, quads;
+    int32_t* table;
+    float* volume;
+    int64_t n;
+};
+
+__global__ __launch_bounds__(256) void lat_build_kernel(const LatBuild b) {
+    const int64_t e = (int64_t)blockIdx.x * blockDim.x + threadIdx.x;
+    if (e >= b.n * b.quads) return;
+    const int64_t i = e / b.quads;
+    const int q = (int)(e - i * b.quads);
+    int c[3];
+    bool in = true;
+#pragma unroll
+    for (int k = 0; k < 3; ++k) {
+        const float r = rintf(__fdiv_rn(__fsub_rn(b.pos[3 * i + k], b.center[k]), b.voxel[k]));
+        in = in && r >= -1.0e9f && r <= 1.0e9f;
+        c[k] = in ? (int)r : 0;
+        in = in && c[k] >= b.bmin[k] && (int64_t)c[k] - b.bmin[k] < b.bdim[k];
+    }
+    if (!in) return;
+    if (b.table && q == 0)
+        b.table[((int64_t)(c[2] - b.bmin[2]) * b.bdim[1] + (c[1] - b.bmin[1])) * b.bdim[0] + (c[0] - b.bmin[0])] = (int32_t)i;
+    if (!b.volume) return;
+    int64_t cell;
+    if (b.split) {
+        const int sub = (c[2] & 1) * 4 + (c[1] & 1) * 2 + (c[0] & 1);
+        cell = (((int64_t)sub * b.hdim[2] + ((c[2] >> 1) - b.hmin[2])) * b.hdim[1] + ((c[1] >> 1) - b.hmin[1])) * b.hdim[0] +
+               ((c[0] >> 1) - b.hmin[0]);
+    } else {
+        cell = ((int64_t)(c[2] - b.bmin[2]) * b.bdim[1] + (c[1] - b.bmin[1])) * b.bdim[0] + (c[0] - b.bmin[0]);
+    }
+    const float* src = b.feat + i * b.C + 4 * q;
+    float* dst = b.volume + cell * b.C + 4 * q;
+    if ((b.C & 3) == 0) {
+        *(f32x4*)dst = *(const f32x4*)src;
+    } else {
+        for (int k = 0; k < 4 && 4 * q + k < b.C; ++k) dst[k] = src[k];
+    }
+}
+
+static int lat_build(const dmcf_lattice_build_args* a, hipStream_t stream) {
+    if (!a || a->n_points < 0 || a->n_points > 0x7fffffff) return DMCF_EINVAL;
+    if (!a->table && !a->volume) return DMCF_EINVAL;
+    if (a->flags & ~DMCF_FLAG_LATTICE_SPLIT) return DMCF_EINVAL;
+    LatBuild b = {};
+    int64_t cells = 1;
+    for (int k = 0; k < 3; ++k) {
+        if (a->box_dims[k] <= 0 || !(a->voxel[k] > 0.0f)) return DMCF_EINVAL;
+        b.voxel[k] = a->voxel[k];
+        b.bmin[k] = a->box_min[k];
+        b.bdim[k] = a->box_dims[k];
+        b.hmin[k] = a->box_min[k] >> 1;
+        b.hdim[k] = (int)(((int64_t)a->box_min[k] + a->box_dims[k] - 1) >> 1) - b.hmin[k] + 1;
+        cells *= a->box_dims[k];
+        if (cells > ((int64_t)1 << 40)) return DMCF_EINVAL;
+    }
+    b.split = (a->flags & DMCF_FLAG_LATTICE_SPLIT) ? 1 : 0;
+    if (a->volume && (a->channels <= 0 || (a->n_points > 0 && !a->features))) return DMCF_EINVAL;
+    if (a->n_points > 0 && (!a->positions || !a->center)) return DMCF_EINVAL;
+    if (a->volume && (((uintptr_t)a->volume | (uintptr_t)a->features) & 15)) return DMCF_EINVAL;
+    const int64_t vcells = b.split ? 8 * (int64_t)b.hdim[0] * b.hdim[1] * b.hdim[2] : cells;
+    if (a->table && hipMemsetAsync(a->table, 0xff, (size_t)cells * 4, stream) != hipSuccess) return check_launch();
+    if (a->volume && hipMemsetAsync(a->volume, 0, (size_t)vcells * a->channels * 4, stream) != hipSuccess) return check_launch();
+    if (a->n_points == 0) return DMCF_OK;
+    b.pos = a->positions; b.center = a->center; b.n = a->n_points;
+    b.table = a->table;
+    b.volume = a->volume; b.feat = a->features; b.C = a->volume ? a->channels : 4;
+    b.quads = (b.C + 3) / 4;
+    const int64_t threads = b.n * b.quads;
+    hipLaunchKernelGGL(lat_build_kernel, dim3((unsigned)((threads + 255) / 256)), dim3(256), 0, stream, b);
+    return check_launch();
+}
 
 }
 
@@ -459,14 +577,14 @@
 
 size_t dmcf_lattice_conv_workspace_bytes(const dmcf_lattice_conv_args* a) {
     if (lat_validate(a) != DMCF_OK) return 256;
-    return lat_layout(a, 1).total;
+    return lat_layout(a, 1, lat_pick_rows(a, 1)).total;
 }
 
 size_t dmcf_lattice_conv_batch_workspace_bytes(const dmcf_lattice_conv_args* parts, int32_t n_parts) {
     if (!parts || n_parts < 1 || n_parts > kLatMaxParts) return 256;
     for (int i = 0; i < n_parts; ++i)
         if (lat_validate(parts + i) != DMCF_OK) return 256;
-    return lat_layout(parts, n_parts).total;
+    return lat_layout(parts, n_parts, lat_pick_rows(parts, n_parts)).total;
 }
 
 int dmcf_lattice_conv_forward(const dmcf_lattice_conv_args* a, void* workspace, size_t workspace_bytes, dmcf_stream_t stream_) {
@@ -480,7 +598,16 @@
     return lat_launch(parts, n_parts, workspace, workspace_bytes, (hipStream_t)stream_);
 }
 
+int dmcf_lattice_build(const dmcf_lattice_build_args* args, dmcf_stream_t stream_) { return lat_build(args, (hipStream_t)stream_); }
+
+static bool lat_any_split(const dmcf_lattice_conv_args* parts, int32_t n_parts) {
+    for (int i = 0; parts && i < n_parts && i < kLatMaxParts; ++i)
+        if (parts[i].flags & (DMCF_FLAG_LATTICE_SPLIT | DMCF_FLAG_FILTER_PACKED)) return true;
+    return false;
+}
+
 size_t dmcf_lattice_conv_backward_workspace_bytes(const dmcf_lattice_conv_args* parts, int32_t n_parts) {
+    if (lat_any_split(parts, n_parts)) return 256;
     dmcf_lattice_conv_args own[kLatMaxParts];
     if (lat_bwd_parts(parts, n_parts, own) != DMCF_OK) return 256;
     return lat_bwd_layout(own, n_parts).total;
@@ -488,6 +615,7 @@
 
 int dmcf_lattice_conv_backward(const dmcf_lattice_conv_args* parts, int32_t n_parts, const float* grad_out, float* grad_volume,
                                float* grad_filters, void* workspace, size_t workspace_bytes, dmcf_stream_t stream_) {
+    if (lat_any_split(parts, n_parts)) return DMCF_EUNSUPPORTED;
     return lat_backward(parts, n_parts, grad_out, grad_volume, grad_filters, workspace, workspace_bytes, (hipStream_t)stream_);
 }
 
diff --git a/dmcf_amd/csrc/misc.hip b/dmcf_amd/csrc/misc.hip
--- a/dmcf_amd/csrc/misc.hip
+++ b/dmcf_amd/csrc/misc.hip
@@ -264,7 +264,7 @@
 
 extern "C" {
 
-int dmcf_version(void) { return 21700; }
+int dmcf_version(void) { return 21800; }
 
 const char* dmcf_error_string(int code) {
     switch (code) {
diff --git a/dmcf_amd/lattice.py b/dmcf_amd/lattice.py
--- a/dmcf_amd/lattice.py
+++ b/dmcf_amd/lattice.py
@@ -176,9 +176,21 @@
         self._core = (lo, [hi[k] - lo[k] for k in range(3)], idx, pos, valid)
         return self._core
 
+    def _native(self, features=None):
+        if not self.gpos.is_cuda:
+            return False
+        return features is None or (features.is_cuda and features.dtype == torch.float32
+                                    and not (torch.is_grad_enabled() and features.requires_grad))
+
+    def _build(self, minp, dims, features=None, table=False, split=False):
+        from . import ops
+        return ops.lattice_build(self.gpos, self.center, self.voxel, minp, dims, features=features, table=table, split=split)
+
     def table_in(self, minp, dims):
         key = (tuple(minp), tuple(dims))
         t = self._tables.get(key)
+        if t is None and self._native():
+            t = self._tables[key] = self._build(minp, dims, table=True)[0]
         if t is None:
             dx, dy, dz = dims
             c = self.cells().long()
@@ -192,7 +204,11 @@
             t = self._tables[key] = t[:-1].view(dz, dy, dx)
         return t
 
-    def volume_in(self, features, minp, dims):
+    def volume_in(self, features, minp, dims, split=False):
+        if self._native(features):
+            return self._build(minp, dims, features=features, split=split)[1]
+        if split:
+            raise ValueError("a volume by cell parity is built on the device only")
         key = ("in", tuple(minp), tuple(dims))
         lin = self._vlin.get(key)
         dx, dy, dz = dims
@@ -208,6 +224,8 @@
         return v[:-1].view(dz, dy, dx, features.shape[1])
 
     def table(self):
+        if self._table is None and self._native():
+            self._table = self._build(self.minp, self.dims, table=True)[0]
         if self._table is None:
             dx, dy, dz = self.dims
             t = torch.full((dz * dy * dx,), -1, dtype=torch.int32, device=self.gpos.device)
@@ -215,7 +233,12 @@
             self._table = t.view(dz, dy, dx)
         return self._table
 
-    def volume(self, features, minp=None, dims=None):
+    def volume(self, features, minp=None, dims=None, split=False):
+        if self._native(features):
+            own = minp is None
+            return self._build(self.minp if own else minp, self.dims if own else dims, features=features, split=split)[1]
+        if split:
+            raise ValueError("a volume by cell parity is built on the device only")
         key = None if minp is None else (tuple(minp), tuple(dims))
         lin = self._vlin.get(key)
         if lin is None:
@@ -315,19 +338,24 @@
         vdim = self.plan(ops, extent, dev)[1]
         return int(vdim[0]) * int(vdim[1]) * int(vdim[2])
 
-    def conv(self, ops, kernel, inp_features, n_out, extent, **kw):
+    def conv(self, ops, kernel, inp_features, n_out, extent, packed_cache=None, **kw):
         a, b = self.inp, self.out
         vmin, vdim, parts = self.plan(ops, extent, inp_features.device)
+        split = (parts is None and int(self.ratio) == 2 and a._native(inp_features) and os.environ.get("DMCF_LATTICE_SPLIT", "1") != "0"
+                 and not (torch.is_grad_enabled() and any(t is not None and t.requires_grad for t in (kernel, kw.get("bias")))))
         if self.cropped:
             omin, odim = b.core()[:2]
-            vol, table, tmin = a.volume_in(inp_features, vmin, vdim), b.table_in(omin, odim), omin
+            vol, table, tmin = a.volume_in(inp_features, vmin, vdim, split=split), b.table_in(omin, odim), omin
             fill = min(1.0, a.gpos.shape[0] / float(max(vdim[0] * vdim[1] * vdim[2], 1)))
         else:
-            vol, table, tmin = a.volume(inp_features, vmin, vdim), b.table(), b.minp
+            vol, table, tmin = a.volume(inp_features, vmin, vdim, split=split), b.table(), b.minp
             fill = a.gpos.shape[0] / float(a.dims[0] * a.dims[1] * a.dims[2])
+        if packed_cache is not None and not (torch.is_grad_enabled() and any(
+                t is not None and t.requires_grad for t in (kernel, inp_features, kw.get("bias")))):
+            kw["packed_cache"] = packed_cache
         if parts is None:
             return ops.lattice_conv(kernel, vol, vmin, table, tmin, n_out, a.voxel, extent, inp_step=int(self.ratio),
-                                    fill=fill, **kw)
+                                    fill=fill, **({"split_dims": vdim} if split else {}), **kw)
         return ops.lattice_conv(kernel, vol, vmin, table, tmin, n_out, a.voxel, extent, inp_step=1, out_stride=2,
                                 parts=parts, fill=fill, **kw)
 
diff --git a/dmcf_amd/ops.py b/dmcf_amd/ops.py
--- a/dmcf_amd/ops.py
+++ b/dmcf_amd/ops.py
@@ -131,6 +131,7 @@
 WINDOWS = {None: 0, "explicit": 1, "poly6": 2, "cubic": 3, "linear": 4, "peak": 5, "cubic_grad": 6}
 
 FLAG_ALIGN_CORNERS, FLAG_NORMALIZE, FLAG_SYMMETRIC, FLAG_ACCUMULATE, FLAG_SKIP_SELF, FLAG_FILTER_PACKED = 1, 2, 4, 8, 16, 32
+FLAG_LATTICE_SPLIT = 64
 
 
 class LaunchTimer:
@@ -586,11 +587,51 @@
     return lo, [hi[k] - lo[k] + 1 for k in range(3)]
 
 
+def lattice_split_dims(box_min, box_dims):
+    hmin = [int(m) >> 1 for m in box_min]
+    return hmin, [((int(m) + int(d) - 1) >> 1) - h + 1 for m, d, h in zip(box_min, box_dims, hmin)]
+
+
+def lattice_build(positions, center, voxel, box_min, box_dims, features=None, table=False, split=False):
+    positions = _dev_f32(positions, "positions", 3)
+    center = _dev_f32(center.reshape(-1), "center")
+    dev = positions.device
+    a = _lib.LatticeBuildArgs()
+    a.positions, a.n_points, a.center = _ptr(positions), int(positions.shape[0]), _ptr(center)
+    for k in range(3):
+        a.voxel[k], a.box_min[k], a.box_dims[k] = float(voxel[k]), int(box_min[k]), int(box_dims[k])
+    dx, dy, dz = (int(d) for d in box_dims)
+    tab = vol = None
+    if table:
+        tab = torch.empty((dz, dy, dx), dtype=torch.int32, device=dev)
+        a.table = _ptr(tab)
+    if features is not None:
+        features = _dev_f32(features, "features")
+        if features.dim() != 2 or features.shape[0] != positions.shape[0]:
+            raise ValueError("features must be [n_points, C]")
+        C = int(features.shape[1])
+        if split:
+            hx, hy, hz = lattice_split_dims(box_min, box_dims)[1]
+            vol = torch.empty((8, hz, hy, hx, C), dtype=torch.float32, device=dev)
+        else:
+            vol = torch.empty((dz, dy, dx, C), dtype=torch.float32, device=dev)
+        a.features, a.channels, a.volume = _ptr(features), C, _ptr(vol)
+        a.flags = FLAG_LATTICE_SPLIT if split else 0
+    _lib.check(_lib.lib().dmcf_lattice_build(ctypes.byref(a), _stream()), "dmcf_lattice_build")
+    return tab, vol
+
+
 def _lattice_args(filters, inp_volume, inp_min, out_table, out_min, n_out, voxel, extent, *, inp_step=1, out_stride=1,
                   out_phase=(0, 0, 0), rel_shift=(0.0, 0.0, 0.0), base_min=None, base_dims=None, window="poly6", window_fac=1.0,
                   align_corners=True, coordinate_mapping="ball_to_cube_volume_preserving", interpolation="linear", bias=None,
-                  out=None, accumulate=False, parts=None):
-    if inp_volume.dim() != 4 or inp_volume.shape[3] != filters.shape[3] or not inp_volume.is_contiguous() or not out_table.is_contiguous():
+                  out=None, accumulate=False, parts=None, split_dims=None):
+    if split_dims is not None:
+        hd = lattice_split_dims(inp_min, split_dims)[1]
+        if tuple(inp_volume.shape) != (8, hd[2], hd[1], hd[0], filters.shape[3]) or not inp_volume.is_contiguous():
+            raise ValueError("a split inp_volume must be a contiguous [8, hz, hy, hx, Cin] tensor (lattice_split_dims)")
+    elif inp_volume.dim() != 4 or inp_volume.shape[3] != filters.shape[3] or not inp_volume.is_contiguous():
+        raise ValueError("inp_volume must be a contiguous [dz, dy, dx, Cin] tensor, out_table a contiguous [dz, dy, dx] one")
+    if not out_table.is_contiguous():
         raise ValueError("inp_volume must be a contiguous [dz, dy, dx, Cin] tensor, out_table a contiguous [dz, dy, dx] one")
     if parts is None:
         parts = [dict(out_phase=out_phase, rel_shift=rel_shift, base_min=base_min, base_dims=base_dims)]
@@ -606,7 +647,7 @@
             a.filter_dims[k] = int(filters.shape[k])
         a.inp_volume, a.out_table = _ptr(inp_volume), _ptr(out_table)
         for k in range(3):
-            a.inp_min[k], a.inp_dims[k] = int(inp_min[k]), int(inp_volume.shape[2 - k])
+            a.inp_min[k], a.inp_dims[k] = int(inp_min[k]), int(inp_volume.shape[2 - k] if split_dims is None else split_dims[k])
             a.out_min[k], a.out_dims[k] = int(out_min[k]), int(out_table.shape[2 - k])
             a.out_phase[k], a.base_min[k], a.base_dims[k] = int(ph[k]), int(bmin[k]), int(bdims[k])
             a.rel_shift[k], a.voxel[k], a.reach[k] = float(sh[k]), float(voxel[k]), reach[k]
@@ -615,7 +656,8 @@
         a.extent, a.window_fac = float(extent), float(window_fac)
         a.window = WINDOWS[window]
         a.coordinate_mapping, a.interpolation = MAPPINGS[coordinate_mapping], INTERPOLATIONS[interpolation]
-        a.flags = (FLAG_ALIGN_CORNERS if align_corners else 0) | (FLAG_ACCUMULATE if accumulate else 0)
+        a.flags = ((FLAG_ALIGN_CORNERS if align_corners else 0) | (FLAG_ACCUMULATE if accumulate else 0) |
+                   (FLAG_LATTICE_SPLIT if split_dims is not None else 0))
         a.bias = _ptr(bias) if bias is not None else None
         a.out = _ptr(out)
         keep.append(offsets)
@@ -626,10 +668,11 @@
 def lattice_conv(filters, inp_volume, inp_min, out_table, out_min, n_out, voxel, extent, inp_step=1, out_stride=1,
                  out_phase=(0, 0, 0), rel_shift=(0.0, 0.0, 0.0), base_min=None, base_dims=None, window="poly6",
                  window_fac=1.0, align_corners=True, coordinate_mapping="ball_to_cube_volume_preserving",
-                 interpolation="linear", bias=None, out=None, accumulate=False, fill=1.0, n_out_launch=None, parts=None):
+                 interpolation="linear", bias=None, out=None, accumulate=False, fill=1.0, n_out_launch=None, parts=None,
+                 split_dims=None, packed_cache=None):
     if torch.is_grad_enabled() and any(t is not None and t.requires_grad for t in (filters, inp_volume, bias)):
-        if out is not None or accumulate:
-            raise ValueError("lattice_conv: out / accumulate cannot be recorded for autograd")
+        if out is not None or accumulate or split_dims is not None:
+            raise ValueError("lattice_conv: out / accumulate / a split volume cannot be recorded for autograd")
         geo = dict(inp_min=inp_min, out_table=out_table, out_min=out_min, n_out=n_out, voxel=voxel, extent=extent,
                    inp_step=inp_step, out_stride=out_stride, out_phase=out_phase, rel_shift=rel_shift, base_min=base_min,
                    base_dims=base_dims, window=window, window_fac=window_fac, align_corners=align_corners,
@@ -647,12 +690,27 @@
                                      out_stride=out_stride, out_phase=out_phase, rel_shift=rel_shift, base_min=base_min,
                                      base_dims=base_dims, window=window, window_fac=window_fac, align_corners=align_corners,
                                      coordinate_mapping=coordinate_mapping, interpolation=interpolation, bias=bias, out=out,
-                                     accumulate=accumulate, parts=parts)
+                                     accumulate=accumulate, parts=parts, split_dims=split_dims)
     if len(arr) == 1:
         nbytes = L.dmcf_lattice_conv_workspace_bytes(arr)
     else:
         nbytes = L.dmcf_lattice_conv_batch_workspace_bytes(arr, len(arr))
-    ws = torch.empty(nbytes, dtype=torch.uint8, device=dev)
+    ws = None
+    if packed_cache is not None:
+        key = (filters._version, tuple(filters.shape), tuple(float(v) for v in voxel), float(extent),
+               tuple((int(a.n_offsets), tuple(a.rel_shift), int(a.offsets or 0)) for a in arr), window, float(window_fac),
+               bool(align_corners), coordinate_mapping, interpolation, str(dev))
+        ws = packed_cache.get("ws")
+        if packed_cache.get("src") is filters and packed_cache.get("key") == key and ws is not None and ws.numel() >= nbytes:
+            for a in arr:
+                a.flags |= FLAG_FILTER_PACKED
+        else:
+            ws = torch.empty(nbytes + nbytes // 4, dtype=torch.uint8, device=dev)
+            packed_cache["key"], packed_cache["ws"], packed_cache["src"] = key, ws, filters
+            packed_cache["keep"] = keep
+        nbytes = ws.numel()
+    if ws is None:
+        ws = torch.empty(nbytes, dtype=torch.uint8, device=dev)
     t0 = timer.begin() if timer is not None else None
     if len(arr) == 1:
         _lib.check(L.dmcf_lattice_conv_forward(arr, _ptr(ws), nbytes, _stream()), "dmcf_lattice_conv_forward")
diff --git a/dmcf_amd/utils/convolutions.py b/dmcf_amd/utils/convolutions.py
--- a/dmcf_amd/utils/convolutions.py
+++ b/dmcf_amd/utils/convolutions.py
@@ -404,16 +404,23 @@
         self.accumulate_into = None
         self.extra_bias = None
         self._packed = {}
+        self._packed_lat = {}
 
     def invalidate_packed(self):
         self._packed.clear()
+        self._packed_lat.clear()
+
+    def _lattice_packed_cache(self):
+        return self._packed_lat if os.environ.get("DMCF_CACHE_PACKED_FILTERS", "1") != "0" else None
 
     def _load_from_state_dict(self, *args, **kwargs):
         self._packed.clear()
+        self._packed_lat.clear()
         return super()._load_from_state_dict(*args, **kwargs)
 
     def build(self, in_channels, device=None):
         self._packed.clear()
+        self._packed_lat.clear()
         device = device or self._device or "cuda"
         self.in_channels = int(in_channels)
         if self.circular:
@@ -501,7 +508,7 @@
             out_features = lat.conv(ops, self.kernel, inp_features, out_positions.shape[0], extent,
                                     window=self.window_function.name, window_fac=self.window_function.fac,
                                     align_corners=self.align_corners, coordinate_mapping=self.coordinate_mapping,
-                                    interpolation=self.interpolation)
+                                    interpolation=self.interpolation, packed_cache=self._lattice_packed_cache())
             return self._train_epilogue(out_features, inp_features, acc, extra_bias)
         if rank1:
             pass
@@ -594,7 +601,7 @@
                     window=self.window_function.name, window_fac=self.window_function.fac,
                     align_corners=self.align_corners, coordinate_mapping=self.coordinate_mapping,
                     interpolation=self.interpolation, bias=self._epilogue_bias(fuse_bias, extra_bias),
-                    out=acc, accumulate=acc is not None)
+                    out=acc, accumulate=acc is not None, packed_cache=self._lattice_packed_cache())
                 stray = lat.strays()
                 if stray is not None:
                     idx_s, pos_s, valid = stray
diff --git a/include/dmcf_hip.h b/include/dmcf_hip.h
--- a/include/dmcf_hip.h
+++ b/include/dmcf_hip.h
@@ -208,12 +208,29 @@
     float* out;
 } dmcf_lattice_conv_args;
 
+#define DMCF_FLAG_LATTICE_SPLIT 64
+
 size_t dmcf_lattice_conv_workspace_bytes(const dmcf_lattice_conv_args* args);
 int dmcf_lattice_conv_forward(const dmcf_lattice_conv_args* args, void* workspace, size_t workspace_bytes,
                               dmcf_stream_t stream);
 size_t dmcf_lattice_conv_batch_workspace_bytes(const dmcf_lattice_conv_args* parts, int32_t n_parts);
 int dmcf_lattice_conv_forward_batch(const dmcf_lattice_conv_args* parts, int32_t n_parts, void* workspace,
                                     size_t workspace_bytes, dmcf_stream_t stream);
+
+typedef struct dmcf_lattice_build_args {
+    const float* positions;
+    int64_t n_points;
+    const float* center;
+    float voxel[3];
+    int32_t box_min[3];
+    int32_t box_dims[3];
+    const float* features;
+    int32_t channels;
+    int32_t flags;
+    int32_t* table;
+    float* volume;
+} dmcf_lattice_build_args;
+int dmcf_lattice_build(const dmcf_lattice_build_args* args, dmcf_stream_t stream);
 
 size_t dmcf_lattice_conv_backward_workspace_bytes(const dmcf_lattice_conv_args* parts, int32_t n_parts);
 int dmcf_lattice_conv_backward(const dmcf_lattice_conv_args* parts, int32_t n_parts, const float* grad_out,
```

After: 13.20 million. 0.987x the previous value.
